# Lu-Zhan/Pano-NeRF

Hardware: AMD Instinct MI355X
Metric: rays/sec (train step) (higher is better)
Workload: dtype f32 (2xfp16 split products, fp32 accumulate; weight-gradient operands h_l / delta_l / r_l / hdot_l stored with 16 significant bits, 'Q24')

## Files before the change

### pano-nerf_amd/csrc/pn_chain.hip

```cpp
#include "pn_common.h"
#include <math.h>
#include <string.h>
#include <stdlib.h>
#include <type_traits>
#include <utility>
#include <vector>

template <typename F, int... Is>
__device__ __forceinline__ void static_for_impl(F&& f, std::integer_sequence<int, Is...>) {
    (f(std::integral_constant<int, Is>{}), ...);
}
template <int N, typename F>
__device__ __forceinline__ void static_for(F&& f) {
    static_for_impl(static_cast<F&&>(f), std::make_integer_sequence<int, N>{});
}

typedef __bf16 bf16x8 __attribute__((ext_vector_type(8)));
typedef _Float16 f16x8 __attribute__((ext_vector_type(8)));
typedef __attribute__((address_space(3))) void* lds_ptr_t;
typedef const __attribute__((address_space(1))) void* gbl_ptr_t;

#ifndef PN_CHAIN_TILE
#define PN_CHAIN_TILE 16
#endif
#ifndef PN_ABL_CHAIN
#define PN_ABL_CHAIN 0
#endif
#define HALF_PI_F 1.5707963705062866f
constexpr int TILE = PN_CHAIN_TILE;
static_assert(TILE == 16 || TILE == 32, "PN_CHAIN_TILE is 16 or 32");
constexpr int NG = 64 / TILE;
constexpr int QB = 4 * NG;
constexpr int KSTEP = 2 * QB;
constexpr int ACCQ = TILE / QB;
constexpr int ACCR = 4 * ACCQ;
#ifndef PN_CHAIN_WAVES
#define PN_CHAIN_WAVES (PN_CHAIN_TILE == 16 ? 8 : 4)
#endif
constexpr int CH_WAVES = PN_CHAIN_WAVES;
constexpr int CH_THREADS = 64 * CH_WAVES;
constexpr int CH_SAMPLES = CH_WAVES * TILE;
constexpr int CH_WG_PER_CU = (TILE == 16 && CH_WAVES == 4) ? 2 : 1;
constexpr int CH_MIN_WAVES = CH_WAVES * CH_WG_PER_CU / 4;
typedef float accv __attribute__((ext_vector_type(ACCR)));
constexpr int KS_H = 256 / KSTEP, NT_H = 256 / TILE;
constexpr int KS_ENC = 96 / KSTEP, NT_ENC = 96 / TILE;
constexpr int KS_PAD = 32 / KSTEP;
constexpr int KS_C = 128 / KSTEP, NT_C = 128 / TILE;

template <int NP>
struct Cfg {
#ifdef PN_CHAIN_CF
    static constexpr int CF = PN_CHAIN_CF;
#else
    static constexpr int CF = NP >= 2 ? 24 : (CH_WG_PER_CU == 2 ? 16 : 32);
#endif
    static constexpr int PER = CF / NP;
    static constexpr int SLOT = (CF + 1) * 1024;
#ifdef PN_CHAIN_NSLOT
    static constexpr int NSLOT = PN_CHAIN_NSLOT;
#else
    static constexpr int NSLOT = CH_WG_PER_CU == 2 ? 3 : (NP >= 2 ? 5 : 4);
#endif
    static constexpr int D = NSLOT - 1;
    static constexpr int SHARE = CF / CH_WAVES;
    static constexpr int LDS_BYTES = SLOT * NSLOT;
};

template <int NP>
struct TEl {
    typedef float type;
};
template <>
struct TEl<1> {
    typedef __bf16 type;
};
#define TP(p) reinterpret_cast<TE*>(p)
template <int NP>
struct PlaneOf {
    typedef bf16x8 type;
};
template <>
struct PlaneOf<2> {
    typedef f16x8 type;
};
template <int NP>
struct BFrag {
    typename PlaneOf<NP>::type p[NP];
};

__host__ __device__ constexpr int feat(int qb, int g, int i) { return QB * qb + 4 * g + i; }
__host__ __device__ constexpr int kmap(int ks, int g, int j) { return feat(2 * ks + (j >> 2), g, j & 3); }

enum {
    F_L0 = 0, F_L1, F_L2, F_L3, F_L4, F_L5, F_L5E, F_L6, F_L7, F_DEN, F_EXTRA, F_VIEW, F_COLOR, F_COUNT
};
enum {
    B_COLOR = 0, B_VIEW, B_EXTRA, B_L7, B_L6, B_L5, B_L4, B_L3, B_L2, B_L1, B_DENC0, B_DENC1, B_COUNT
};
__host__ __device__ constexpr int fwd_ks(int i) {
    return (i == F_L0 || i == F_L5E) ? KS_ENC : i == F_VIEW ? KS_H + KS_PAD : i == F_COLOR ? KS_C : KS_H;
}
__host__ __device__ constexpr int fwd_nt(int i) { return (i == F_DEN || i == F_COLOR) ? 1 : i == F_VIEW ? NT_C : NT_H; }
__host__ __device__ constexpr int bwd_ks(int i) {
    return i == B_COLOR ? 1 : i == B_VIEW ? KS_C : i == B_EXTRA ? KS_H + 1 : KS_H;
}
__host__ __device__ constexpr int bwd_nt(int i) { return i == B_COLOR ? NT_C : (i == B_DENC0 || i == B_DENC1) ? NT_ENC : NT_H; }
template <int NP>
__host__ __device__ constexpr int chunks_of(int KS, int NT) { return (KS * NT + Cfg<NP>::PER - 1) / Cfg<NP>::PER; }
template <int NP>
__host__ __device__ constexpr int fwd_chunk0(int i) {
    int c = 0;
    for (int k = 0; k < i; ++k) c += chunks_of<NP>(fwd_ks(k), fwd_nt(k));
    return c;
}
template <int NP>
__host__ __device__ constexpr int bwd_chunk0(int i) {
    int c = 0;
    for (int k = 0; k < i; ++k) c += chunks_of<NP>(bwd_ks(k), bwd_nt(k));
    return c;
}

struct PackSeg {
    int64_t off;
    int ld;
    int k0, kvalid;
    int transposed;
    int col0;
};
struct PackLayer {
    int chunk0, KS, NT;
    int rows_valid;
    int nseg;
    PackSeg seg[2];
    int64_t aux_off;
    int aux_n;
};
#define PACK_MAXL 32
struct PackTable {
    PackLayer L[PACK_MAXL];
    int n, nchunks;
};

constexpr int EXP_TOP = 15;
constexpr int EXP_CAP = 80;
constexpr int EXP_CAP_W = 30;
constexpr int EXP_CAP_Z = 120;
__device__ __forceinline__ int scale_exp(float amax, int cap = EXP_CAP) {
    const int e = EXP_TOP - __builtin_amdgcn_frexp_expf(amax);
    return e > cap ? cap : e;
}
constexpr int WEXP_SLICES = 16;
__global__ void k_chain_wexp(PackTable tab, const float* params, uint32_t* wmax) {
    const PackLayer& L = tab.L[blockIdx.x];
    float m = 0.f;
    for (int s = 0; s < L.nseg; ++s) {
        const PackSeg& sg = L.seg[s];
        const int n = L.rows_valid * sg.kvalid;
        for (int idx = threadIdx.x + blockDim.x * blockIdx.y; idx < n; idx += blockDim.x * WEXP_SLICES) {
            const int i = idx / sg.kvalid, kr = idx - i * sg.kvalid;
            const float x = sg.transposed ? params[sg.off + (int64_t)kr * sg.ld + sg.col0 + i]
                                          : params[sg.off + (int64_t)i * sg.ld + sg.col0 + kr];
            m = fmaxf(m, fabsf(x));
        }
    }
    __shared__ float red[256];
    red[threadIdx.x] = m;
    __syncthreads();
    for (int o = 128; o > 0; o >>= 1) {
        if ((int)threadIdx.x < o) red[threadIdx.x] = fmaxf(red[threadIdx.x], red[threadIdx.x + o]);
        __syncthreads();
    }
    if (threadIdx.x == 0) wmax[blockIdx.x * WEXP_SLICES + blockIdx.y] = __float_as_uint(red[0]);
}

template <int NP>
__global__ void k_chain_pack(PackTable tab, const float* params, unsigned char* out, int* wexp) {
    constexpr int CF = Cfg<NP>::CF, SLOT = Cfg<NP>::SLOT, PER = Cfg<NP>::PER;
    const int64_t gid = (int64_t)blockIdx.x * blockDim.x + threadIdx.x;
    const int lane = (int)(gid & 63);
    const int64_t fi = gid >> 6;
    const int chunk = (int)(fi / (CF + 1)), f = (int)(fi % (CF + 1));
    if (chunk >= tab.nchunks) return;
    int li = 0;
    for (int i = 1; i < tab.n; ++i)
        if (chunk >= tab.L[i].chunk0) li = i;
    const PackLayer& L = tab.L[li];
    unsigned char* dst = out + (int64_t)chunk * SLOT + f * 1024 + lane * 16;
    if (f == CF) {
        float v[4] = {0.f, 0.f, 0.f, 0.f};
        if (chunk == L.chunk0 + (L.KS * L.NT + PER - 1) / PER - 1 && L.aux_off >= 0)
            for (int q = 0; q < 4; ++q)
                if (lane * 4 + q < L.aux_n) v[q] = params[L.aux_off + lane * 4 + q];
        memcpy(dst, v, 16);
        return;
    }
    const int p = f % NP;
    const int step = (chunk - L.chunk0) * PER + f / NP;
    int wex = 0;
    if constexpr (NP == 2) {
        const uint32_t* wm = reinterpret_cast<const uint32_t*>(wexp) + 32 + li * WEXP_SLICES;
        uint32_t top = 0u;
#pragma unroll
        for (int sl = 0; sl < WEXP_SLICES; ++sl) top = wm[sl] > top ? wm[sl] : top;
        wex = scale_exp(__uint_as_float(top), EXP_CAP_W);
        if (chunk == L.chunk0 && f == 0 && lane == 0) wexp[li] = wex;
    }
    unsigned short o[8] = {0, 0, 0, 0, 0, 0, 0, 0};
    if (step < L.KS * L.NT) {
        const int ks = step / L.NT, tt = step % L.NT;
        const int i = TILE * tt + (lane % TILE), g = lane / TILE;
        for (int j = 0; j < 8; ++j) {
            const int k = kmap(ks, g, j);
            float x = 0.f;
            if (i < L.rows_valid)
                for (int s = 0; s < L.nseg; ++s) {
                    const PackSeg& sg = L.seg[s];
                    const int kr = k - sg.k0;
                    if (kr >= 0 && kr < sg.kvalid)
                        x = sg.transposed ? params[sg.off + (int64_t)kr * sg.ld + sg.col0 + i]
                                          : params[sg.off + (int64_t)i * sg.ld + sg.col0 + kr];
                }
            unsigned short bits;
            if constexpr (NP == 2) {
                const float t = ldexpf(x, wex);
                const _Float16 hh = (_Float16)t;
                const _Float16 r = p == 0 ? hh : (_Float16)(t - (float)hh);
                __builtin_memcpy(&bits, &r, 2);
            } else {
                const __bf16 hb = (__bf16)x;
                __bf16 r = hb;
                if (p >= 1) {
                    const float r1 = x - (float)hb;
                    const __bf16 mb = (__bf16)r1;
                    r = mb;
                    if (p == 2) r = (__bf16)(r1 - (float)mb);
                }
                __builtin_memcpy(&bits, &r, 2);
            }
            o[j] = bits;
        }
    }
    memcpy(dst, o, 16);
}

#if defined(PN_TRACE_CHAIN) || defined(PN_TRACE_WG)
__device__ unsigned long long g_chain_trace[64];
extern "C" int pn_chain_trace_read(unsigned long long* out) {
    return hipMemcpyFromSymbol(out, HIP_SYMBOL(g_chain_trace), sizeof(unsigned long long) * 64) == hipSuccess ? 0 : -4;
}
#endif
#ifdef PN_TRACE_CHAIN
#define TR(i)                                                                                          \
    do {                                                                                               \
        if (blockIdx.x == 0 && threadIdx.x == 0 && st == (int64_t)gridDim.x) g_chain_trace[i] = __builtin_amdgcn_s_memtime(); \
    } while (0)
#define TRX(i)                                                                                 \
    do {                                                                                       \
        if (blockIdx.x == 0 && threadIdx.x == 0) g_chain_trace[i] = __builtin_amdgcn_s_memtime(); \
    } while (0)
#else
#define TR(i)
#define TRX(i)
#endif

template <int NP>
struct Ring {
    static constexpr int CF = Cfg<NP>::CF, SLOT = Cfg<NP>::SLOT;
    static constexpr int PIECES = CF / CH_WAVES + 1;
    __amdgpu_buffer_rsrc_t rsrc;
    unsigned char* lds;
    uint32_t lds_addr;
    int nchunk;
    int pf, pslot, cslot;
    int wid, lane;
    int cur_soff;
    unsigned char* cur_lds;
    __device__ __forceinline__ void begin_round() {
        cur_soff = pf * SLOT;
        cur_lds = lds + pslot * SLOT;
        pf = (pf + 1 == nchunk) ? 0 : pf + 1;
        pslot = (pslot + 1 == Cfg<NP>::NSLOT) ? 0 : pslot + 1;
    }
    template <int I, bool AUX>
    __device__ __forceinline__ void piece() {
        if constexpr (I < CF / CH_WAVES) {
            const int f = wid + CH_WAVES * I;
            __builtin_amdgcn_raw_ptr_buffer_load_lds(rsrc, (lds_ptr_t)(cur_lds + f * 1024), 16, lane * 16, cur_soff + f * 1024, 0, 0);
        } else if constexpr (I == CF / CH_WAVES && AUX) {
            if (wid < 4) {
                const int o = CF * 1024 + wid * 256;
                __builtin_amdgcn_raw_ptr_buffer_load_lds(rsrc, (lds_ptr_t)(cur_lds + o), 4, lane * 4, cur_soff + o, 0, 0);
            }
        }
    }
    template <int I0, int STRIDE, bool AUX = true>
    __device__ __forceinline__ void pieces_from() {
        if constexpr (I0 < PIECES) {
            piece<I0, AUX>();
            pieces_from<I0 + STRIDE, STRIDE, AUX>();
        }
    }
    __device__ __forceinline__ void start(const unsigned char* s, unsigned char* l, int n, int w, int ln, int first) {
        rsrc = __builtin_amdgcn_make_buffer_rsrc((void*)s, 0, n * SLOT, 0x00020000);
        lds = l; nchunk = n; wid = w; lane = ln;
        lds_addr = (uint32_t)(uintptr_t)(lds_ptr_t)l;
        pf = first; pslot = 0; cslot = 0;
#pragma unroll
        for (int i = 0; i < Cfg<NP>::D; ++i) {
            begin_round();
            pieces_from<0, 1, true>();
        }
    }
#ifdef PN_TRACE_CHAIN
    unsigned long long t_lds = 0, t_dma = 0, t_bar = 0, n_acq = 0;
#endif
    __device__ __forceinline__ uint32_t acquire() {
        constexpr int N = Cfg<NP>::SHARE * (Cfg<NP>::D - 1);
#ifdef PN_TRACE_CHAIN
        const unsigned long long t0 = __builtin_amdgcn_s_memtime();
        asm volatile("s_waitcnt lgkmcnt(0)" ::: "memory");
        const unsigned long long t1 = __builtin_amdgcn_s_memtime();
        asm volatile("s_waitcnt vmcnt(%0) lgkmcnt(0)" ::"n"(N) : "memory");
        const unsigned long long t2 = __builtin_amdgcn_s_memtime();
        __builtin_amdgcn_s_barrier();
        const unsigned long long t3 = __builtin_amdgcn_s_memtime();
        asm volatile("s_waitcnt lgkmcnt(0)" ::: "memory");
        t_lds += t1 - t0; t_dma += t2 - t1; t_bar += t3 - t2; ++n_acq;
#else
        asm volatile("s_waitcnt vmcnt(%0) lgkmcnt(0)" ::"n"(N) : "memory");
        if constexpr (!(PN_ABL_CHAIN & 8)) __builtin_amdgcn_s_barrier();
#endif
        begin_round();
        const uint32_t p = lds_addr + cslot * SLOT;
        cslot = (cslot + 1 == Cfg<NP>::NSLOT) ? 0 : cslot + 1;
        return p;
    }
    __device__ __forceinline__ void drain() {
        asm volatile("s_waitcnt vmcnt(0)" ::: "memory");
        __builtin_amdgcn_s_barrier();
#ifdef PN_TRACE_CHAIN
        if (blockIdx.x == 0 && threadIdx.x == 0) {
            g_chain_trace[56] = t_lds; g_chain_trace[57] = t_dma; g_chain_trace[58] = t_bar; g_chain_trace[59] = n_acq;
        }
#endif
    }
};

__device__ __forceinline__ void chain_prio(int wid) {
#ifdef PN_CHAIN_PRIO
    if (wid >= CH_WAVES / 2) __builtin_amdgcn_s_setprio(PN_CHAIN_PRIO);
#endif
}

__device__ __forceinline__ accv mfma1(const bf16x8& a, const bf16x8& b, accv v) {
#if PN_CHAIN_TILE == 32
    return __builtin_amdgcn_mfma_f32_32x32x16_bf16(a, b, v, 0, 0, 0);
#else
    return __builtin_amdgcn_mfma_f32_16x16x32_bf16(a, b, v, 0, 0, 0);
#endif
}
__device__ __forceinline__ accv mfma1(const f16x8& a, const f16x8& b, accv v) {
#if PN_CHAIN_TILE == 32
    return __builtin_amdgcn_mfma_f32_32x32x16_f16(a, b, v, 0, 0, 0);
#else
    return __builtin_amdgcn_mfma_f32_16x16x32_f16(a, b, v, 0, 0, 0);
#endif
}
template <int NP>
__device__ __forceinline__ accv mfma_split(const BFrag<NP>& a, const BFrag<NP>& b, accv v) {
    if constexpr (NP == 3) {
        v = mfma1(a.p[2], b.p[0], v);
        v = mfma1(a.p[0], b.p[2], v);
        v = mfma1(a.p[1], b.p[1], v);
        v = mfma1(a.p[1], b.p[0], v);
        v = mfma1(a.p[0], b.p[1], v);
        v = mfma1(a.p[0], b.p[0], v);
    } else if constexpr (NP == 2) {
        v = mfma1(a.p[1], b.p[0], v);
        v = mfma1(a.p[0], b.p[1], v);
        v = mfma1(a.p[0], b.p[0], v);
    } else {
        v = mfma1(a.p[0], b.p[0], v);
    }
    return v;
}

template <int NP, int IDX>
__device__ __forceinline__ void read_a(BFrag<NP>& a, uint32_t addr) {
#pragma unroll
    for (int p = 0; p < NP; ++p)
        asm volatile("ds_read_b128 %0, %1 offset:%2" : "=v"(a.p[p]) : "v"(addr), "n"((IDX * NP + p) * 1024) : "memory");
}
template <int NP, int LEFT>
__device__ __forceinline__ void wait_a(BFrag<NP>& a) {
    if constexpr (NP == 3)
        asm volatile("s_waitcnt lgkmcnt(%3)" : "+v"(a.p[0]), "+v"(a.p[1]), "+v"(a.p[2]) : "n"(LEFT) : "memory");
    else if constexpr (NP == 2)
        asm volatile("s_waitcnt lgkmcnt(%2)" : "+v"(a.p[0]), "+v"(a.p[1]) : "n"(LEFT) : "memory");
    else
        asm volatile("s_waitcnt lgkmcnt(%1)" : "+v"(a.p[0]) : "n"(LEFT) : "memory");
}
template <int NP, int NT>
struct Unit {
    static constexpr int U = 1;
};
template <int NP>
struct Look {
    static constexpr int N = NP == 3 ? 1 : 3;
};
template <int NP>
__host__ __device__ constexpr int chunk_steps(int S, int c) {
    return (c == (S - 1) / Cfg<NP>::PER && S % Cfg<NP>::PER) ? S % Cfg<NP>::PER : Cfg<NP>::PER;
}
template <int NP, int S, int PP>
__device__ __forceinline__ void read_step(Ring<NP>& R, uint32_t& sa, int lane, BFrag<NP>& f) {
    if constexpr (PP < S) {
        if constexpr (PP % Cfg<NP>::PER == 0) sa = R.acquire() + lane * 16;
        if constexpr (PN_ABL_CHAIN & 2) f = BFrag<NP>{};
        else read_a<NP, PP % Cfg<NP>::PER>(f, sa);
    }
}
template <int NP, int S, int PP, bool BIASNEXT>
__device__ __forceinline__ void piece_step(Ring<NP>& R) {
    if constexpr (PP < S && !(PN_ABL_CHAIN & 1)) {
        constexpr int PER = Cfg<NP>::PER, c = PP / PER, n = (S + PER - 1) / PER;
        R.template pieces_from<PP % PER, chunk_steps<NP>(S, c), true>();
    }
}
template <int NP>
__device__ __forceinline__ void tie(BFrag<NP>& a) {
    if constexpr (NP == 3) asm volatile("" : "+v"(a.p[0]), "+v"(a.p[1]), "+v"(a.p[2]));
    else if constexpr (NP == 2) asm volatile("" : "+v"(a.p[0]), "+v"(a.p[1]));
    else asm volatile("" : "+v"(a.p[0]));
}
__device__ __forceinline__ void mfma_pair(const BFrag<2>& a0, const BFrag<2>& a1, const BFrag<2>& b, accv& v0, accv& v1) {
    v0 = mfma1(a0.p[1], b.p[0], v0);
    v1 = mfma1(a1.p[1], b.p[0], v1);
    v0 = mfma1(a0.p[0], b.p[1], v0);
    v1 = mfma1(a1.p[0], b.p[1], v1);
    v0 = mfma1(a0.p[0], b.p[0], v0);
    v1 = mfma1(a1.p[0], b.p[0], v1);
}
template <int NP, int KS, int NT, int S0, bool BIASNEXT, bool ZERO = false>
struct GemmStep {
    static constexpr int LA = Look<NP>::N, U = Unit<NP, NT>::U;
    static_assert(LA >= U && LA % U == 0 && (KS * NT) % U == 0, "look-ahead in whole units");
    static __device__ __forceinline__ void run(Ring<NP>& R, const BFrag<NP> (&b)[KS], accv (&acc)[NT], uint32_t& sa,
                                               BFrag<NP> (&q)[LA], int lane) {
        constexpr int S = KS * NT;
        constexpr int hi = (S0 + LA + U) < S ? (S0 + LA + U) : S;
        constexpr int young = hi > S0 + U ? hi - (S0 + U) : 0;
        BFrag<NP> nw[U];
        read_step<NP, S, S0 + LA>(R, sa, lane, nw[0]);
        if constexpr (U == 2) read_step<NP, S, S0 + LA + 1>(R, sa, lane, nw[1]);
        wait_a<NP, NP * young>(q[0]);
        constexpr int ks = S0 / NT, t = S0 % NT;
        if constexpr (U == 2) {
            tie<NP>(q[1]);
            mfma_pair(q[0], q[1], b[ks], acc[t], acc[t + 1]);
        } else if constexpr (!(PN_ABL_CHAIN & 4)) {
            if constexpr (ZERO && ks == 0) {
                accv z;
#pragma unroll
                for (int e = 0; e < ACCR; ++e) z[e] = 0.f;
                acc[t] = mfma_split<NP>(q[0], b[ks], z);
            } else {
                acc[t] = mfma_split<NP>(q[0], b[ks], acc[t]);
            }
        }
#ifdef PN_ABL_FILL
        {
            float f0 = __int_as_float(lane), f1 = f0;
#pragma unroll
            for (int k = 0; k < PN_ABL_FILL; ++k) asm volatile("v_fma_f32 %0, %1, %1, %0" : "+v"(f0) : "v"(f1));
            asm volatile("" ::"v"(f0));
        }
#endif
        __builtin_amdgcn_sched_barrier(0);
        piece_step<NP, S, S0 + LA, BIASNEXT>(R);
        if constexpr (U == 2) piece_step<NP, S, S0 + LA + 1, BIASNEXT>(R);
        __builtin_amdgcn_sched_barrier(0);
        if constexpr (S0 + U < S) {
#pragma unroll
            for (int i = 0; i + U < LA; ++i) q[i] = q[i + U];
#pragma unroll
            for (int u = 0; u < U; ++u) q[LA - U + u] = nw[u];
            GemmStep<NP, KS, NT, S0 + U, BIASNEXT, ZERO>::run(R, b, acc, sa, q, lane);
        }
    }
};
template <int NP, int S, int I, bool BIASNEXT>
__device__ __forceinline__ void gemm_prologue(Ring<NP>& R, uint32_t sa, BFrag<NP> (&q)[Look<NP>::N]) {
    if constexpr (I < Look<NP>::N && I < S) {
        read_a<NP, I>(q[I], sa);
        piece_step<NP, S, I, BIASNEXT>(R);
        gemm_prologue<NP, S, I + 1, BIASNEXT>(R, sa, q);
    }
}
template <int NP, int KS, int NT, bool BIAS, bool ZERO, bool BIASNEXT = false>
__device__ __forceinline__ void chain_gemm(Ring<NP>& R, const BFrag<NP> (&b)[KS], accv (&acc)[NT], int lane, int sc = 0) {
    constexpr int CF = Cfg<NP>::CF;
    static_assert(Look<NP>::N <= Cfg<NP>::PER, "the look-ahead stays within one chunk boundary");
    const uint32_t s0 = R.acquire();
    if constexpr (!ZERO && NP == 2) {
#pragma unroll
        for (int t = 0; t < NT; ++t)
#pragma unroll
            for (int e = 0; e < ACCR; ++e) {
                const float x = acc[t][e];
                acc[t][e] = ldexpf(x, sc);
            }
    }
    uint32_t sa = s0 + lane * 16;
    BFrag<NP> q[Look<NP>::N];
    gemm_prologue<NP, KS * NT, 0, BIASNEXT>(R, sa, q);
    GemmStep<NP, KS, NT, 0, BIASNEXT, ZERO>::run(R, b, acc, sa, q, lane);
    if constexpr (BIAS) {
        const float* aux = reinterpret_cast<const float*>(R.lds + ((sa - lane * 16) - R.lds_addr) + CF * 1024) + 4 * (lane / TILE);
        const float inv = NP == 2 ? ldexpf(1.0f, -sc) : 1.0f;
#pragma unroll
        for (int t = 0; t < NT; ++t)
#pragma unroll
            for (int qd = 0; qd < ACCQ; ++qd) {
                const f32x4 v = *reinterpret_cast<const f32x4*>(aux + QB * (ACCQ * t + qd));
#pragma unroll
                for (int i = 0; i < 4; ++i) {
                    const float x = acc[t][4 * qd + i];
                    acc[t][4 * qd + i] = NP == 2 ? __builtin_fmaf(x, inv, v[i]) : x + v[i];
                }
            }
    } else if constexpr (NP == 2) {
#pragma unroll
        for (int t = 0; t < NT; ++t)
#pragma unroll
            for (int e = 0; e < ACCR; ++e) {
                const float x = acc[t][e];
                acc[t][e] = ldexpf(x, -sc);
            }
    }
}

__device__ __forceinline__ void split2_pair(float x0, float x1, float s, uint32_t& h, uint32_t& l) {
    asm("v_fma_mixlo_f16 %0, %1, %2, 0" : "=v"(h) : "v"(x0), "v"(s));
    asm("v_fma_mixhi_f16 %0, %1, %2, 0" : "+v"(h) : "v"(x1), "v"(s));
    asm("v_fma_mixlo_f16 %0, %1, %2, -%3 op_sel_hi:[0,0,1]" : "=v"(l) : "v"(x0), "v"(s), "v"(h));
    asm("v_fma_mixhi_f16 %0, %1, %2, -%3 op_sel:[0,0,1] op_sel_hi:[0,0,1]" : "+v"(l) : "v"(x1), "v"(s), "v"(h));
}
template <int N>
__device__ __forceinline__ void split2_pairs(const float (&x)[2 * N], float s, uint32_t (&h)[N], uint32_t (&l)[N]) {
#pragma unroll
    for (int q = 0; q < N; ++q) asm("v_fma_mixlo_f16 %0, %1, %2, 0" : "=v"(h[q]) : "v"(x[2 * q]), "v"(s));
#pragma unroll
    for (int q = 0; q < N; ++q) asm("v_fma_mixhi_f16 %0, %1, %2, 0" : "+v"(h[q]) : "v"(x[2 * q + 1]), "v"(s));
#pragma unroll
    for (int q = 0; q < N; ++q)
        asm("v_fma_mixlo_f16 %0, %1, %2, -%3 op_sel_hi:[0,0,1]" : "=v"(l[q]) : "v"(x[2 * q]), "v"(s), "v"(h[q]));
#pragma unroll
    for (int q = 0; q < N; ++q)
        asm("v_fma_mixhi_f16 %0, %1, %2, -%3 op_sel:[0,0,1] op_sel_hi:[0,0,1]" : "+v"(l[q]) : "v"(x[2 * q + 1]), "v"(s), "v"(h[q]));
}
__device__ __forceinline__ float pow2f(int e) { return __int_as_float((127 + e) << 23); }
template <int NP>
__device__ __forceinline__ void split_into(const float (&x)[8], BFrag<NP>& f, int ex = 0) {
    if constexpr (NP == 2) {
        typedef uint32_t u32x4 __attribute__((ext_vector_type(4)));
        const float s = pow2f(ex);
        uint32_t hq[4], lq[4];
        split2_pairs<4>(x, s, hq, lq);
        u32x4 h, l;
#pragma unroll
        for (int q = 0; q < 4; ++q) {
            h[q] = hq[q];
            l[q] = lq[q];
        }
        f.p[0] = __builtin_bit_cast(f16x8, h);
        f.p[1] = __builtin_bit_cast(f16x8, l);
    }
    if constexpr (NP != 2) {
#pragma unroll
        for (int j = 0; j < 8; ++j) {
            const __bf16 h = (__bf16)x[j];
            f.p[0][j] = h;
            if constexpr (NP == 3) {
                const float r1 = x[j] - (float)h;
                const __bf16 m = (__bf16)r1;
                f.p[1][j] = m;
                f.p[2][j] = (__bf16)(r1 - (float)m);
            }
        }
    }
}
struct Ex {
    int ex;
    uint32_t top;
};
__device__ __forceinline__ void swap32(uint32_t x, uint32_t& a, uint32_t& b) {
    const auto r = __builtin_amdgcn_permlane32_swap(x, x, false, false);
    a = r[0];
    b = r[1];
}
__device__ __forceinline__ void swap16(uint32_t x, uint32_t& a, uint32_t& b) {
    const auto r = __builtin_amdgcn_permlane16_swap(x, x, false, false);
    a = r[0];
    b = r[1];
}
__device__ __forceinline__ float col_max(float m) {
    uint32_t a, b;
    swap32(__float_as_uint(m), a, b);
    uint32_t u = a > b ? a : b;
    if constexpr (NG == 4) {
        swap16(u, a, b);
        u = a > b ? a : b;
    }
    return __uint_as_float(u);
}
__device__ __forceinline__ float col_sum(float v) {
    uint32_t a, b;
    swap32(__float_as_uint(v), a, b);
    v = __uint_as_float(a) + __uint_as_float(b);
    if constexpr (NG == 4) {
        swap16(__float_as_uint(v), a, b);
        v = __uint_as_float(a) + __uint_as_float(b);
    }
    return v;
}
__device__ __forceinline__ uint32_t row_umax(uint32_t v) {
    uint32_t o;
    o = (uint32_t)__builtin_amdgcn_update_dpp(0, (int)v, 0xB1, 0xF, 0xF, true);
    v = v > o ? v : o;
    o = (uint32_t)__builtin_amdgcn_update_dpp(0, (int)v, 0x4E, 0xF, 0xF, true);
    v = v > o ? v : o;
    o = (uint32_t)__builtin_amdgcn_update_dpp(0, (int)v, 0x141, 0xF, 0xF, true);
    v = v > o ? v : o;
    o = (uint32_t)__builtin_amdgcn_update_dpp(0, (int)v, 0x140, 0xF, 0xF, true);
    v = v > o ? v : o;
    return v;
}
__device__ __forceinline__ Ex ex_of(float lane_max, int cap = EXP_CAP) {
    const float cm = col_max(lane_max);
    Ex e;
    e.ex = scale_exp(cm, cap);
    uint32_t v = row_umax(__float_as_uint(cm));
    if constexpr (NG == 2) {
        const uint32_t o = (uint32_t)__shfl_xor((int)v, 16, 64);
        v = v > o ? v : o;
    }
    e.top = (uint32_t)__builtin_amdgcn_readfirstlane((int)v);
    return e;
}
template <int N>
struct RunMax {
    uint32_t v[N];
    __device__ __forceinline__ void clear() {
#pragma unroll
        for (int k = 0; k < N; ++k) v[k] = 0u;
    }
    __device__ __forceinline__ void upd(int idx, uint32_t x) {
#pragma unroll
        for (int k = 0; k < N; ++k) v[k] = (idx == k && x > v[k]) ? x : v[k];
    }
    __device__ __forceinline__ void flush(uint32_t* slots, int lane, int wid, unsigned char* lds) const {
        if (!slots) return;
        uint32_t* w = reinterpret_cast<uint32_t*>(lds);
        if (lane == 0) {
#pragma unroll
            for (int k = 0; k < N; ++k) w[wid * N + k] = v[k];
        }
        __syncthreads();
        if (wid == 0 && lane < N) {
            uint32_t m = w[lane];
#pragma unroll
            for (int i = 1; i < CH_WAVES; ++i) m = m > w[i * N + lane] ? m : w[i * N + lane];
            if (m > __atomic_load_n(slots + lane, __ATOMIC_RELAXED)) atomicMax(slots + lane, m);
        }
    }
};
enum {
    AM_ENC = 0, AM_ACT0 = 1 , AM_DELTA0 = 11 ,
    AM_D8B = 19, AM_D8D = 20, AM_DHV = 21, AM_DRGB = 22, AM_RS0 = 23 , AM_TANG0 = 31 ,
    AM_EDOT = 39, AM_COEF = 40, AM_COUNT = 64
};
template <int NT>
__device__ __forceinline__ float lane_amax(const accv (&acc)[NT]) {
    float m[4] = {0.f, 0.f, 0.f, 0.f};
#pragma unroll
    for (int t = 0; t < NT; ++t)
#pragma unroll
        for (int e = 0; e < ACCR; ++e) {
            const float x = acc[t][e];
            m[e & 3] = fmaxf(m[e & 3], fabsf(x));
        }
    return fmaxf(fmaxf(m[0], m[1]), fmaxf(m[2], m[3]));
}
#define AQ(acc, qb, i) (acc)[(qb) / ACCQ][4 * ((qb) % ACCQ) + (i)]
template <int NP, int NT, int KB>
__device__ __forceinline__ void split_acc(const accv (&acc)[NT], BFrag<NP> (&b)[KB], int ex) {
#pragma unroll
    for (int s = 0; s < NT * ACCQ / 2; ++s) {
        float x[8];
#pragma unroll
        for (int j = 0; j < 8; ++j) x[j] = AQ(acc, 2 * s + (j >> 2), j & 3);
        split_into<NP>(x, b[s], ex);
    }
}
template <int NP, int NT, int KB>
__device__ __forceinline__ Ex acc_to_b(const accv (&acc)[NT], BFrag<NP> (&b)[KB], float also = 0.f, int cap = EXP_CAP) {
    constexpr int KS = NT * ACCQ / 2;
    static_assert((NT * ACCQ) % 2 == 0 && KS <= KB, "quad blocks");
    Ex e{0, 0u};
    if constexpr (NP == 2) e = ex_of(fmaxf(lane_amax<NT>(acc), also), cap);
    split_acc<NP, NT, KB>(acc, b, e.ex);
    return e;
}
#ifndef PN_T_NT
#define PN_T_NT 1
#endif
template <int NT, typename TE>
__device__ __forceinline__ void store_t(TE* base, const accv (&acc)[NT]) {
    if constexpr (PN_ABL_CHAIN & 16) return;
#pragma unroll
    for (int qb = 0; qb < NT * ACCQ; ++qb)
#pragma unroll
        for (int i = 0; i < 4; ++i) {
            const float x = AQ(acc, qb, i);
#if PN_T_NT
            __builtin_nontemporal_store((TE)x, base + (QB * qb + i) * TILE);
#else
            base[(QB * qb + i) * TILE] = (TE)x;
#endif
        }
}

#ifndef PN_NO_Q24
#define PN_NO_Q24 0
#endif
template <int NP>
constexpr bool kQ24 = (NP == 2 && TILE == 16 && !PN_NO_Q24);
__host__ __device__ constexpr bool q24_act(int slot) { return slot <= 6; }
__host__ __device__ constexpr bool q24_delta(int slot) { return slot != 0 && slot != 5; }
typedef uint32_t u32x3 __attribute__((ext_vector_type(3)));
__device__ __forceinline__ u32x3 pack_q24(float x0, float x1, float x2, float x3) {
    const uint32_t e0 = __float_as_uint(x0) + 0x80u, e1 = __float_as_uint(x1) + 0x80u;
    const uint32_t e2 = __float_as_uint(x2) + 0x80u, e3 = __float_as_uint(x3) + 0x80u;
    u32x3 v;
    v[0] = __builtin_amdgcn_perm(e1, e0, 0x05030201u);
    v[1] = __builtin_amdgcn_perm(e2, e1, 0x06050302u);
    v[2] = __builtin_amdgcn_perm(e3, e2, 0x07060503u);
    return v;
}
__device__ __forceinline__ int q24_lane(int c, int g) { return g * 192 + c * 12; }
#ifndef PN_Q24_NT
#define PN_Q24_NT 1
#endif
template <int NT>
__device__ __forceinline__ void store_q24(unsigned char* base, const accv (&acc)[NT]) {
    if constexpr (PN_ABL_CHAIN & 16) return;
#pragma unroll
    for (int qb = 0; qb < NT * ACCQ; ++qb)
#if PN_Q24_NT
        __builtin_nontemporal_store(pack_q24(AQ(acc, qb, 0), AQ(acc, qb, 1), AQ(acc, qb, 2), AQ(acc, qb, 3)), reinterpret_cast<u32x3*>(base + qb * 768));
#else
        *reinterpret_cast<u32x3*>(base + qb * 768) = pack_q24(AQ(acc, qb, 0), AQ(acc, qb, 1), AQ(acc, qb, 2), AQ(acc, qb, 3));
#endif
}

constexpr int MW = 4 / (NG / 2);
__host__ __device__ constexpr int gate_word(int ks, int j) { return (4 * ks + (j >> 1)) >> 4; }
__host__ __device__ constexpr int gate_bit(int ks, int j) { return ((4 * ks + (j >> 1)) & 15) + 16 * (j & 1); }
struct Gate {
    uint32_t w[MW];
};
template <int NT>
__device__ __forceinline__ void relu(accv (&acc)[NT]) {
#pragma unroll
    for (int t = 0; t < NT; ++t)
#pragma unroll
        for (int e = 0; e < ACCR; ++e) {
            const float x = acc[t][e];
            acc[t][e] = fmaxf(x, 0.f);
        }
}
template <int NP, int KS, int KB>
__device__ __forceinline__ void gate_words(const BFrag<NP> (&b)[KB], Gate& g) {
    typedef uint32_t u32x4 __attribute__((ext_vector_type(4)));
#pragma unroll
    for (int i = 0; i < MW; ++i) g.w[i] = 0u;
    uint32_t one = 0x00010001u;
    asm volatile("" : "+v"(one));
#pragma unroll
    for (int ks = 0; ks < KS; ++ks) {
        const u32x4 h = __builtin_bit_cast(u32x4, b[ks].p[0]);
#pragma unroll
        for (int q = 0; q < 4; ++q) {
            const uint32_t hq = h[q];
            uint32_t m;
            asm("v_pk_min_u16 %0, %1, %2" : "=v"(m) : "v"(hq), "v"(one));
            asm("v_lshl_or_b32 %0, %1, %2, %0" : "+v"(g.w[(4 * ks + q) >> 4]) : "v"(m), "n"((4 * ks + q) & 15));
        }
    }
}
template <int NT>
__device__ __forceinline__ void gate_bits(accv (&acc)[NT], const Gate& g) {
#pragma unroll
    for (int qb = 0; qb < NT * ACCQ; ++qb)
#pragma unroll
        for (int i = 0; i < 4; ++i) {
            const int ks = qb >> 1, j = 4 * (qb & 1) + i;
            const int m = __builtin_amdgcn_sbfe((int)g.w[gate_word(ks, j)], gate_bit(ks, j), 1);
            const float x = AQ(acc, qb, i);
            AQ(acc, qb, i) = __int_as_float(__float_as_int(x) & m);
        }
}
__device__ __forceinline__ Gate load_gate(const uint32_t* masks, int64_t slot, int64_t Mp, int64_t row, int g) {
    Gate r;
    const uint32_t* p = masks + ((slot * Mp + row) * 8 + MW * g);
    if constexpr (MW == 4) {
        const uint4 v = *reinterpret_cast<const uint4*>(p);
        r.w[0] = v.x; r.w[1] = v.y; r.w[2] = v.z; r.w[3] = v.w;
    } else {
        const uint2 v = *reinterpret_cast<const uint2*>(p);
        r.w[0] = v.x; r.w[1] = v.y;
    }
    return r;
}
__device__ __forceinline__ void store_gate(uint32_t* masks, int64_t slot, int64_t Mp, int64_t row, int g, const Gate& r) {
    uint32_t* p = masks + ((slot * Mp + row) * 8 + MW * g);
    if constexpr (MW == 4) *reinterpret_cast<uint4*>(p) = make_uint4(r.w[0], r.w[1], r.w[2], r.w[3]);
    else *reinterpret_cast<uint2*>(p) = make_uint2(r.w[0], r.w[1]);
}
template <int N>
__device__ __forceinline__ Gate pop_front(Gate (&q)[N]) {
    const Gate m = q[0];
#pragma unroll
    for (int i = 0; i + 1 < N; ++i) q[i] = q[i + 1];
    return m;
}


__device__ __forceinline__ float ch_sp_d1(float x) { return x > 20.f ? 1.f : 1.f / (1.f + expf(-x)); }
__device__ __forceinline__ float ch_sp_d2(float x) {
    if (x > 20.f) return 0.f;
    const float s = 1.f / (1.f + expf(-x));
    return s * (1.f - s);
}
__device__ __forceinline__ float sel3(const float (&v)[3], int ch) { return ch == 0 ? v[0] : (ch == 1 ? v[1] : v[2]); }

__device__ __forceinline__ float red_turns(float y, int& quadrant) {
    const float c_hi = 0.15915494f;
    const float c_lo = 6.4206382e-9f;
    const float p = y * c_hi;
    float e = __builtin_fmaf(y, c_hi, -p);
    e = __builtin_fmaf(y, c_lo, e);
    const float f = (p - __builtin_rintf(p)) + e;
    const float q4 = f * 4.0f;
    const float qn = __builtin_rintf(q4);
    quadrant = (int)qn;
    return (q4 - qn) * 1.5707963267948966f;
}
__device__ __forceinline__ float ksin(float x) {
    const float z = x * x;
    float p = __builtin_fmaf(z, 2.7557319e-6f, -1.9841270e-4f);
    p = __builtin_fmaf(z, p, 8.3333333e-3f);
    p = __builtin_fmaf(z, p, -1.6666667e-1f);
    return __builtin_fmaf(x * z, p, x);
}
__device__ __forceinline__ float kcos(float x) {
    const float z = x * x;
    float p = __builtin_fmaf(z, -2.7557319e-7f, 2.4801587e-5f);
    p = __builtin_fmaf(z, p, -1.3888889e-3f);
    p = __builtin_fmaf(z, p, 4.1666667e-2f);
    p = __builtin_fmaf(z, p, -0.5f);
    return __builtin_fmaf(z, p, 1.0f);
}
__device__ __forceinline__ float fast_sin(float y) {
    int q;
    const float r = red_turns(y, q);
    const float sv = ksin(r), cv = kcos(r);
    const float v = (q & 1) ? cv : sv;
    return (q & 2) ? -v : v;
}
__device__ __forceinline__ float fast_cos(float y) {
    int q;
    const float r = red_turns(y, q);
    const float sv = ksin(r), cv = kcos(r);
    const float v = (q & 1) ? sv : cv;
    return ((q + 1) & 2) ? -v : v;
}

__device__ __forceinline__ int opaque(int v) {
    asm volatile("" : "+v"(v));
    return v;
}
__device__ __forceinline__ void level_of(int f, int& l, int& ch) {
    l = (f * 43691) >> 17;
    ch = f - 3 * l;
}
__device__ __forceinline__ float pow2i(int l) { return __int_as_float((127 + l) << 23); }

struct Tile {
    int64_t blk, row, rc;
    int c, g, lo;
    bool live;
};
__device__ __forceinline__ Tile tile_of(int64_t st, int wid, int lane, int64_t M) {
    Tile t;
    t.c = lane % TILE;
    t.g = lane / TILE;
    t.blk = st * CH_WAVES + wid;
    t.row = t.blk * TILE + t.c;
    t.live = t.row < M;
    t.rc = t.live ? t.row : M - 1;
    t.lo = t.c + 4 * t.g * TILE;
    return t;
}
template <int NP, int NT>
__device__ __forceinline__ void store_vec(typename TEl<NP>::type* slot, const Tile& T, int F, bool q, const accv (&acc)[NT]) {
    if constexpr (kQ24<NP>) {
        if (q) {
            store_q24<NT>(reinterpret_cast<unsigned char*>(slot) + T.blk * (int64_t)(F * TILE * 3) + opaque(q24_lane(T.c, T.g)), acc);
            return;
        }
    }
    store_t<NT>(slot + T.blk * (int64_t)(F * TILE) + opaque(T.lo), acc);
}

template <int NP, int MODE>
__device__ __forceinline__ Ex encode(const float (&mu)[3], const float (&cv)[3], const float (&vv)[3], int g,
                                      typename TEl<NP>::type* et, BFrag<NP> (&benc)[KS_ENC]) {
    typedef typename TEl<NP>::type TE;
    constexpr int NQ = 96 / QB;
    float x[NQ][4];
    const int g4 = 4 * opaque(g);
#pragma unroll
    for (int qb = 0; qb < NQ / 2; ++qb)
#pragma unroll
        for (int i = 0; i < 4; ++i) {
            int l, ch;
            level_of(QB * qb + g4 + i, l, ch);
            const float sc = pow2i(l);
            const float y = sel3(mu, ch) * sc;
            const float e0 = __expf(-0.5f * (sel3(cv, ch) * (sc * sc)));
            if constexpr (MODE == 0) {
                x[qb][i] = e0 * fast_sin(y);
                x[qb + NQ / 2][i] = e0 * fast_sin(y + HALF_PI_F);
            } else {
                const float e = e0 * sc * sel3(vv, ch);
                x[qb][i] = e * fast_cos(y);
                x[qb + NQ / 2][i] = e * fast_cos(y + HALF_PI_F);
            }
        }
#ifdef PN_TRACE_CHAIN
#pragma unroll
    for (int qb = 0; qb < NQ; ++qb)
#pragma unroll
        for (int i = 0; i < 4; ++i) asm volatile("" ::"v"(x[qb][i]));
    if (MODE == 0) TRX(31);
#endif
#pragma unroll
    for (int qb = 0; qb < NQ; ++qb)
#pragma unroll
        for (int i = 0; i < 4; ++i) et[(QB * qb + i) * TILE] = (TE)x[qb][i];
    if (MODE == 0) TRX(32);
    Ex e{0, 0u};
    if constexpr (NP == 2) {
        if constexpr (MODE == 0) {
            e.ex = EXP_TOP - 1;
            e.top = 0x3f800000u;
        } else {
            float m = 0.f;
#pragma unroll
            for (int qb = 0; qb < NQ; ++qb)
#pragma unroll
                for (int i = 0; i < 4; ++i) m = fmaxf(m, fabsf(x[qb][i]));
            e = ex_of(m, EXP_CAP_Z);
        }
    }
#pragma unroll
    for (int s = 0; s < KS_ENC; ++s) {
        float y8[8];
#pragma unroll
        for (int j = 0; j < 8; ++j) y8[j] = x[2 * s + (j >> 2)][j & 3];
        split_into<NP>(y8, benc[s], e.ex);
    }
    return e;
}
template <int NP, int KS>
__device__ __forceinline__ int reload_b(const typename TEl<NP>::type* src, BFrag<NP> (&b)[KS], int cap = EXP_CAP) {
    if constexpr (NP == 2) {
        float x[KS][8];
        float m = 0.f;
#pragma unroll
        for (int ks = 0; ks < KS; ++ks)
#pragma unroll
            for (int j = 0; j < 8; ++j) {
                x[ks][j] = (float)src[(QB * (2 * ks + (j >> 2)) + (j & 3)) * TILE];
                m = fmaxf(m, fabsf(x[ks][j]));
            }
        const int ex = scale_exp(col_max(m), cap);
#pragma unroll
        for (int ks = 0; ks < KS; ++ks) split_into<NP>(x[ks], b[ks], ex);
        return ex;
    } else {
#pragma unroll
        for (int ks = 0; ks < KS; ++ks) {
            float x[8];
#pragma unroll
            for (int j = 0; j < 8; ++j) x[j] = (float)src[(QB * (2 * ks + (j >> 2)) + (j & 3)) * TILE];
            split_into<NP>(x, b[ks]);
        }
        return 0;
    }
}
__device__ __forceinline__ void ipe_backward_tiles(const accv (&acc)[NT_ENC], const float (&mu)[3], const float (&cv)[3], int g,
                                                   float (&dm)[3]) {
    dm[0] = dm[1] = dm[2] = 0.f;
    const int g4 = 4 * opaque(g);
#pragma unroll
    for (int qb = 0; qb < 96 / QB; ++qb)
#pragma unroll
        for (int i = 0; i < 4; ++i) {
            const bool cosine = qb >= 96 / QB / 2;
            int l, ch;
            level_of(QB * (cosine ? qb - 96 / QB / 2 : qb) + g4 + i, l, ch);
            const float sc = pow2i(l);
            const float y = sel3(mu, ch) * sc;
            const float ex = __expf(-0.5f * (sel3(cv, ch) * (sc * sc))) * sc;
            const float d = AQ(acc, qb, i) * ex * fast_cos(cosine ? y + HALF_PI_F : y);
            dm[0] += ch == 0 ? d : 0.f;
            dm[1] += ch == 1 ? d : 0.f;
            dm[2] += ch == 2 ? d : 0.f;
        }
#pragma unroll
    for (int i = 0; i < 3; ++i) {
        dm[i] = col_sum(dm[i]);
    }
}
template <int NP>
__device__ __forceinline__ Ex finish_gated(accv (&acc)[NT_H], const Gate& m, typename TEl<NP>::type* slot, const Tile& T, bool q24,
                                           BFrag<NP> (&bh)[KS_H]) {
    gate_bits<NT_H>(acc, m);
    if (slot) store_vec<NP, NT_H>(slot, T, 256, q24, acc);
    return acc_to_b<NP, NT_H, KS_H>(acc, bh, 0.f, EXP_CAP_Z);
}

__global__ void k_view_table(int64_t view_rows, const float* viewdirs, float* tab, uint32_t* amax, int amax_n) {
    if (amax && blockIdx.x == 0 && (int)threadIdx.x < amax_n) amax[threadIdx.x] = 0u;
    const int64_t idx = (int64_t)blockIdx.x * blockDim.x + threadIdx.x;
    if (idx >= view_rows * 32) return;
    const int64_t r = idx >> 5;
    const int v = (int)(idx & 31);
    const float vd0 = viewdirs[r * 3], vd1 = viewdirs[r * 3 + 1], vd2 = viewdirs[r * 3 + 2];
    auto vsel = [&](int ch) { return ch == 0 ? vd0 : (ch == 1 ? vd1 : vd2); };
    const int i = v - 3, half = i >= 12 ? 1 : 0;
    int l, ch;
    level_of(i < 0 ? 0 : i - 12 * half, l, ch);
    const float xb = vsel(ch) * pow2i(l & 3);
    const float sv = fast_sin(half ? xb + HALF_PI_F : xb);
    tab[idx] = v < 3 ? vsel(v) : (v < PN_VIEW_DIM ? sv : 0.f);
}

struct FwdArgs {
    int64_t M, nst;
    int rows_per_ray, nc;
    int64_t view_rows;
    const unsigned char* pack;
    const int* wexp;
    uint32_t* amax;
    const float* mean;
    const float* cov;
    const float* viewdirs;
    float* view_tab;
    float* enc_t;
    float* acts_t;
    uint32_t* masks;
    float* raw_rgb;
    float* raw_den;
    int q24;
};
__host__ __device__ constexpr int64_t act_off(int slot, int64_t Mp) {
    return slot <= 8 ? (int64_t)slot * Mp * 256 : 8 * Mp * 256 + Mp * 288;
}
__host__ __device__ constexpr int64_t acts_floats(int64_t Mp) { return 8 * Mp * 256 + Mp * 288 + Mp * 128; }

template <int NP>
__global__ __launch_bounds__(CH_THREADS, CH_MIN_WAVES) void k_chain_fwd(FwdArgs a) {
    extern __shared__ __attribute__((aligned(16))) unsigned char lds[];
    typedef typename TEl<NP>::type TE;
    const int tid = threadIdx.x, lane = tid & 63;
    const int wid = __builtin_amdgcn_readfirstlane(tid >> 6);
    const int64_t Mp = a.nst * CH_SAMPLES;
    chain_prio(wid);
    Ring<NP> R;
    R.start(a.pack, lds, fwd_chunk0<NP>(F_COUNT), wid, lane, 0);
    RunMax<10> RM;
    RM.clear();
#ifdef PN_TRACE_CHAIN
    if (blockIdx.x == 0 && threadIdx.x == 0) {
        g_chain_trace[60] = __builtin_amdgcn_s_memtime();
        g_chain_trace[61] = __builtin_amdgcn_s_memrealtime();
    }
#endif
    int wtab = 0;
    if constexpr (NP == 2) wtab = a.wexp[lane & 15];
    for (int64_t st = blockIdx.x; st < a.nst; st += gridDim.x) {
        const Tile T = tile_of(st, wid, lane, a.M);
        TR(0);
        TE* et = TP(a.enc_t) + T.blk * (96 * TILE) + T.lo;
        BFrag<NP> bh[KS_H];
        accv acc[NT_H];
        Gate mw;
        int bex = 0;
        auto wx = [&](int i) {
            if constexpr (NP == 2) return __builtin_amdgcn_readlane(wtab, i);
            else return 0;
        };
        {
            float mu[3], cv[3];
            const float zero3[3] = {0.f, 0.f, 0.f};
#pragma unroll
            for (int i = 0; i < 3; ++i) {
                mu[i] = a.mean[T.rc * 3 + i];
                cv[i] = a.cov[T.rc * 3 + i];
            }
            BFrag<NP> benc[KS_ENC];
#ifdef PN_TRACE_CHAIN
            asm volatile("" ::"v"(mu[0]), "v"(mu[1]), "v"(mu[2]), "v"(cv[0]), "v"(cv[1]), "v"(cv[2]));
            TRX(30);
#endif
            bex = encode<NP, 0>(mu, cv, zero3, T.g, et, benc).ex;
            TR(1);
            chain_gemm<NP, KS_ENC, NT_H, true, true, true>(R, benc, acc, lane, wx(F_L0) + bex);
            TR(2);
        }
        auto finish_hidden = [&](int slot) {
            relu<NT_H>(acc);
            if (TP(a.acts_t)) store_vec<NP, NT_H>(TP(a.acts_t) + act_off(slot, Mp), T, 256, a.q24 && q24_act(slot), acc);
            const Ex e = acc_to_b<NP, NT_H, KS_H>(acc, bh);
            gate_words<NP, KS_H, KS_H>(bh, mw);
            store_gate(a.masks, slot, Mp, T.blk * TILE + T.c, T.g, mw);
            bex = e.ex;
            RM.upd(slot, e.top);
        };
        finish_hidden(0);
        TR(3);
#pragma unroll 1
        for (int l = 1; l <= 4; ++l) {
            chain_gemm<NP, KS_H, NT_H, true, true, true>(R, bh, acc, lane, wx(F_L0 + l) + bex);
            TR(2 + 2 * l);
            finish_hidden(l);
            TR(3 + 2 * l);
        }
        {
            chain_gemm<NP, KS_H, NT_H, false, true, true>(R, bh, acc, lane, wx(F_L5) + bex);
            BFrag<NP> benc[KS_ENC];
            const int eex = reload_b<NP, KS_ENC>(et, benc);
            chain_gemm<NP, KS_ENC, NT_H, true, false, true>(R, benc, acc, lane, wx(F_L5E) + eex);
            TR(12);
            finish_hidden(5);
            TR(13);
        }
#pragma unroll 1
        for (int l = 6; l <= 7; ++l) {
            chain_gemm<NP, KS_H, NT_H, true, true, true>(R, bh, acc, lane, wx(F_L6 + l - 6) + bex);
            TR(2 + 2 * l);
            finish_hidden(l);
            TR(3 + 2 * l);
        }
        {
            accv ad[1];
            chain_gemm<NP, KS_H, 1, true, true, true>(R, bh, ad, lane, wx(F_DEN) + bex);
            if (T.live) {
#pragma unroll
                for (int i = 0; i < 4; ++i) {
                    const int ch = 4 * T.g + i;
                    if (ch < a.nc) a.raw_den[T.row * a.nc + ch] = ad[0][i];
                }
            }
        }
        TR(18);
        BFrag<NP> bv[KS_H + KS_PAD];
        int vex;
        {
            chain_gemm<NP, KS_H, NT_H, true, true, true>(R, bh, acc, lane, wx(F_EXTRA) + bex);
            TR(19);
            TE* bt = a.acts_t ? TP(a.acts_t) + act_off(8, Mp) + T.blk * (288 * TILE) + T.lo : nullptr;
            if (bt) store_t<NT_H>(bt, acc);
            const Ex e = acc_to_b<NP, NT_H, KS_H + KS_PAD>(acc, bv, 1.0f);
            vex = e.ex;
            RM.upd(8, e.top);
            const float* vt = a.view_tab + ((T.rc / a.rows_per_ray) % a.view_rows) * 32 + 4 * T.g;
#pragma unroll
            for (int q = 0; q < KS_PAD; ++q) {
                float x[8];
#pragma unroll
                for (int h = 0; h < 2; ++h) {
                    const f32x4 v = *reinterpret_cast<const f32x4*>(vt + QB * (2 * q + h));
#pragma unroll
                    for (int i = 0; i < 4; ++i) {
                        x[4 * h + i] = v[i];
                        if (bt) bt[(256 + QB * (2 * q + h) + i) * TILE] = (TE)v[i];
                    }
                }
                split_into<NP>(x, bv[KS_H + q], vex);
            }
        }
        TR(20);
        BFrag<NP> bc[KS_C];
        int cex;
        {
            accv av[NT_C];
            chain_gemm<NP, KS_H + KS_PAD, NT_C, true, true, true>(R, bv, av, lane, wx(F_VIEW) + vex);
            TR(21);
            Gate w4;
            relu<NT_C>(av);
            if (TP(a.acts_t)) store_t<NT_C>(TP(a.acts_t) + act_off(9, Mp) + T.blk * (128 * TILE) + T.lo, av);
            const Ex e = acc_to_b<NP, NT_C, KS_C>(av, bc);
            gate_words<NP, KS_C, KS_C>(bc, w4);
            store_gate(a.masks, 8, Mp, T.blk * TILE + T.c, T.g, w4);
            cex = e.ex;
            RM.upd(9, e.top);
        }
        TR(22);
        {
            accv ac[1];
            chain_gemm<NP, KS_C, 1, true, true, true>(R, bc, ac, lane, wx(F_COLOR) + cex);
            TR(23);
            if (T.live && T.g == 0) {
#pragma unroll
                for (int e = 0; e < 3; ++e) a.raw_rgb[T.row * 3 + e] = ac[0][e];
            }
        }
        TR(24);
    }
    R.drain();
#ifdef PN_TRACE_CHAIN
    if (blockIdx.x == 0 && threadIdx.x == 0) {
        g_chain_trace[62] = __builtin_amdgcn_s_memtime();
        g_chain_trace[63] = __builtin_amdgcn_s_memrealtime();
    }
#endif
    if constexpr (NP == 2) {
        RM.flush(a.amax ? a.amax + AM_ACT0 : nullptr, lane, wid, lds);
        if (a.amax && blockIdx.x == 0 && tid == 0) a.amax[AM_ENC] = 0x3f800000u;
    }
}

struct SweepArgs {
    int64_t M, nst;
    int nc;
    float density_bias;
    const unsigned char* pack;
    int nchunk;
    const int* wexp;
    uint32_t* amax;
    const uint32_t* masks;
    const float* raw_den;
    const float* mean;
    const float* cov;
    const float* wd0;
    const float* v;
    float* vec_t;
    int keep_all;
    float* edot_t;
    float* out3;
    float* sdot;
    int q24;
};

template <int NP>
__global__ __launch_bounds__(CH_THREADS, CH_MIN_WAVES) void k_chain_dgrad(SweepArgs a) {
    extern __shared__ __attribute__((aligned(16))) unsigned char lds[];
    typedef typename TEl<NP>::type TE;
    const int tid = threadIdx.x, lane = tid & 63;
    const int wid = __builtin_amdgcn_readfirstlane(tid >> 6);
    const int64_t Mp = a.nst * CH_SAMPLES;
    chain_prio(wid);
    Ring<NP> R;
    R.start(a.pack, lds, a.nchunk, wid, lane, 0);
    RunMax<8> RM;
    RM.clear();
    int wtab = 0;
    if constexpr (NP == 2) wtab = a.wexp[lane & 15];
    for (int64_t st = blockIdx.x; st < a.nst; st += gridDim.x) {
        const Tile T = tile_of(st, wid, lane, a.M);
        Gate mk[8];
#pragma unroll
        for (int l = 0; l < 8; ++l) mk[l] = load_gate(a.masks, 7 - l, Mp, T.blk * TILE + T.c, T.g);
        float mu[3], cv[3];
#pragma unroll
        for (int i = 0; i < 3; ++i) {
            mu[i] = a.mean[T.rc * 3 + i];
            cv[i] = a.cov[T.rc * 3 + i];
        }
        const float sgm = T.live ? ch_sp_d1(a.raw_den[T.rc * a.nc] + a.density_bias) : 0.f;
        BFrag<NP> bh[KS_H];
        int bex = 0;
        auto wx = [&](int i) {
            if constexpr (NP == 2) return __builtin_amdgcn_readlane(wtab, i);
            else return 0;
        };
        {
            const bool Q7 = kQ24<NP> && a.q24 && q24_delta(7);
            TE* rt = (a.keep_all && !Q7) ? TP(a.vec_t) + (int64_t)7 * Mp * 256 + T.blk * (256 * TILE) + T.lo : nullptr;
            unsigned char* rq = (a.keep_all && Q7) ? reinterpret_cast<unsigned char*>(TP(a.vec_t) + (int64_t)7 * Mp * 256) +
                                                         T.blk * (int64_t)(256 * TILE * 3) + q24_lane(T.c, T.g)
                                                   : nullptr;
            const Gate m7 = pop_front(mk);
            if constexpr (NP == 2) {
                float wm = 0.f;
#pragma unroll
                for (int qb = 0; qb < NT_H * ACCQ; ++qb) {
                    const f32x4 wv = *reinterpret_cast<const f32x4*>(a.wd0 + QB * qb + 4 * T.g);
                    wm = fmaxf(fmaxf(wm, fmaxf(fabsf(wv[0]), fabsf(wv[1]))), fmaxf(fabsf(wv[2]), fabsf(wv[3])));
                }
                const Ex e = ex_of(sgm * wm, EXP_CAP_Z);
                bex = e.ex;
                RM.upd(7, e.top);
            }
#pragma unroll
            for (int ks = 0; ks < KS_H; ++ks) {
                float x[8];
#pragma unroll
                for (int h = 0; h < 2; ++h) {
                    const f32x4 wv = *reinterpret_cast<const f32x4*>(a.wd0 + QB * (2 * ks + h) + 4 * T.g);
#pragma unroll
                    for (int i = 0; i < 4; ++i) {
                        const int j = 4 * h + i;
                        const uint32_t bit = (m7.w[gate_word(ks, j)] >> gate_bit(ks, j)) & 1u;
                        x[j] = bit ? sgm * wv[i] : 0.f;
                        if (rt) rt[(QB * (2 * ks + h) + i) * TILE] = (TE)x[j];
                    }
                    if constexpr (kQ24<NP>) {
                        if (rq) {
#if PN_Q24_NT
                            __builtin_nontemporal_store(pack_q24(x[4 * h], x[4 * h + 1], x[4 * h + 2], x[4 * h + 3]), reinterpret_cast<u32x3*>(rq + (2 * ks + h) * 768));
#else
                            *reinterpret_cast<u32x3*>(rq + (2 * ks + h) * 768) = pack_q24(x[4 * h], x[4 * h + 1], x[4 * h + 2], x[4 * h + 3]);
#endif
                        }
                    }
                }
                split_into<NP>(x, bh[ks], bex);
            }
        }
        accv acc[NT_H];
#pragma unroll 1
        for (int l = 7; l >= 1; --l) {
            chain_gemm<NP, KS_H, NT_H, false, true>(R, bh, acc, lane, wx(B_L7 + 7 - l) + bex);
            TE* dst = a.keep_all ? TP(a.vec_t) + (int64_t)(l - 1) * Mp * 256 : (l - 1 == 5 ? TP(a.vec_t) : nullptr);
            const Ex e = finish_gated<NP>(acc, pop_front(mk), dst, T, a.q24 && q24_delta(l - 1), bh);
            bex = e.ex;
            RM.upd(l - 1, e.top);
        }
        {
            accv a3[NT_ENC];
            chain_gemm<NP, KS_H, NT_ENC, false, true>(R, bh, a3, lane, wx(B_DENC0) + bex);
            bex = reload_b<NP, KS_H>(TP(a.vec_t) + (a.keep_all ? (int64_t)5 * Mp * 256 : 0) + T.blk * (256 * TILE) + T.lo, bh, EXP_CAP_Z);
            chain_gemm<NP, KS_H, NT_ENC, false, false>(R, bh, a3, lane, wx(B_DENC1) + bex);
            float dm[3];
            ipe_backward_tiles(a3, mu, cv, T.g, dm);
            if (T.live && T.g == 0) {
                a.out3[T.row * 3] = dm[0];
                a.out3[T.row * 3 + 1] = dm[1];
                a.out3[T.row * 3 + 2] = dm[2];
            }
        }
    }
    R.drain();
    if constexpr (NP == 2) RM.flush(a.amax ? a.amax + AM_RS0 : nullptr, lane, wid, lds);
}

template <int NP>
__global__ __launch_bounds__(CH_THREADS, CH_MIN_WAVES) void k_chain_tangent(SweepArgs a) {
    extern __shared__ __attribute__((aligned(16))) unsigned char lds[];
    typedef typename TEl<NP>::type TE;
    const int tid = threadIdx.x, lane = tid & 63;
    const int wid = __builtin_amdgcn_readfirstlane(tid >> 6);
    const int64_t Mp = a.nst * CH_SAMPLES;
    chain_prio(wid);
    Ring<NP> R;
    R.start(a.pack, lds, a.nchunk, wid, lane, 0);
    RunMax<9> RM;
    RM.clear();
    Ex e;
    int wtab = 0;
    if constexpr (NP == 2) wtab = a.wexp[lane & 15];
    for (int64_t st = blockIdx.x; st < a.nst; st += gridDim.x) {
        const Tile T = tile_of(st, wid, lane, a.M);
        Gate mk[8];
#pragma unroll
        for (int l = 0; l < 8; ++l) mk[l] = load_gate(a.masks, l, Mp, T.blk * TILE + T.c, T.g);
        TE* et = TP(a.edot_t) + T.blk * (96 * TILE) + T.lo;
        BFrag<NP> bh[KS_H];
        accv acc[NT_H];
        int bex = 0;
        auto wx = [&](int i) {
            if constexpr (NP == 2) return __builtin_amdgcn_readlane(wtab, i);
            else return 0;
        };
        {
            float mu[3], cv[3], vv[3];
#pragma unroll
            for (int i = 0; i < 3; ++i) {
                mu[i] = a.mean[T.rc * 3 + i];
                cv[i] = a.cov[T.rc * 3 + i];
                vv[i] = T.live ? a.v[T.rc * 3 + i] : 0.f;
            }
            BFrag<NP> benc[KS_ENC];
            e = encode<NP, 1>(mu, cv, vv, T.g, et, benc);
            bex = e.ex;
            RM.upd(8, e.top);
            chain_gemm<NP, KS_ENC, NT_H, false, true>(R, benc, acc, lane, wx(F_L0) + bex);
        }
        e = finish_gated<NP>(acc, pop_front(mk), TP(a.vec_t), T, a.q24 && q24_act(0), bh);
        bex = e.ex;
        RM.upd(0, e.top);
#pragma unroll 1
        for (int l = 1; l <= 4; ++l) {
            chain_gemm<NP, KS_H, NT_H, false, true>(R, bh, acc, lane, wx(F_L0 + l) + bex);
            e = finish_gated<NP>(acc, pop_front(mk), TP(a.vec_t) + (int64_t)l * Mp * 256, T, a.q24 && q24_act(l), bh);
            bex = e.ex;
            RM.upd(l, e.top);
        }
        {
            chain_gemm<NP, KS_H, NT_H, false, true>(R, bh, acc, lane, wx(F_L5) + bex);
            BFrag<NP> benc[KS_ENC];
            const int eex = reload_b<NP, KS_ENC>(et, benc, EXP_CAP_Z);
            chain_gemm<NP, KS_ENC, NT_H, false, false>(R, benc, acc, lane, wx(F_L5E) + eex);
            e = finish_gated<NP>(acc, pop_front(mk), TP(a.vec_t) + (int64_t)5 * Mp * 256, T, a.q24 && q24_act(5), bh);
            bex = e.ex;
            RM.upd(5, e.top);
        }
        chain_gemm<NP, KS_H, NT_H, false, true>(R, bh, acc, lane, wx(F_L6) + bex);
        e = finish_gated<NP>(acc, pop_front(mk), TP(a.vec_t) + (int64_t)6 * Mp * 256, T, a.q24 && q24_act(6), bh);
        bex = e.ex;
        RM.upd(6, e.top);
        chain_gemm<NP, KS_H, NT_H, false, true>(R, bh, acc, lane, wx(F_L7) + bex);
        {
            gate_bits<NT_H>(acc, pop_front(mk));
            store_t<NT_H>(TP(a.vec_t) + (int64_t)7 * Mp * 256 + T.blk * (256 * TILE) + T.lo, acc);
            if constexpr (NP == 2) RM.upd(7, ex_of(lane_amax<NT_H>(acc), EXP_CAP_Z).top);
            float sd = 0.f;
#pragma unroll
            for (int qb = 0; qb < NT_H * ACCQ; ++qb) {
                const f32x4 wv = *reinterpret_cast<const f32x4*>(a.wd0 + QB * qb + 4 * T.g);
#pragma unroll
                for (int i = 0; i < 4; ++i) sd += AQ(acc, qb, i) * wv[i];
            }
            sd = col_sum(sd);
            if (T.live && T.g == 0) a.sdot[T.row] = sd;
        }
    }
    R.drain();
    if constexpr (NP == 2) RM.flush(a.amax ? a.amax + AM_TANG0 : nullptr, lane, wid, lds);
}

struct BwdArgs {
    int64_t M, nst;
    int nc;
    float density_bias;
    const unsigned char* pack;
    int nchunk;
    const int* wexp;
    uint32_t* amax;
    const uint32_t* masks;
    const float* raw_den;
    const float* d_rgb;
    const float* d_den;
    const float* sdot;
    const float* mean;
    const float* cov;
    float* drgb_t;
    float* dhv_t;
    float* d8_t;
    float* delta_t;
    float* coef_t;
    float* d_mean;
    int q24;
};

template <int NP>
__global__ __launch_bounds__(CH_THREADS, CH_MIN_WAVES) void k_chain_bwd(BwdArgs a) {
    extern __shared__ __attribute__((aligned(16))) unsigned char lds[];
    typedef typename TEl<NP>::type TE;
    const int tid = threadIdx.x, lane = tid & 63;
    const int wid = __builtin_amdgcn_readfirstlane(tid >> 6);
    const int64_t Mp = a.nst * CH_SAMPLES;
    chain_prio(wid);
    Ring<NP> R;
    R.start(a.pack, lds, a.nchunk, wid, lane, 0);
    RunMax<12> RM;
    RM.clear();
    Ex e;
    int wtab = 0;
    if constexpr (NP == 2) wtab = a.wexp[lane & 15];
    for (int64_t st = blockIdx.x; st < a.nst; st += gridDim.x) {
        const Tile T = tile_of(st, wid, lane, a.M);
        Gate mk[9];
#pragma unroll
        for (int l = 0; l < 9; ++l) mk[l] = load_gate(a.masks, 8 - l, Mp, T.blk * TILE + T.c, T.g);
        BFrag<NP> b1[1];
        int bex = 0;
        auto wx = [&](int i) {
            if constexpr (NP == 2) return __builtin_amdgcn_readlane(wtab, i);
            else return 0;
        };
        {
            float x[8];
            TE* dt = TP(a.drgb_t) + T.blk * (32 * TILE) + T.lo;
            float m = 0.f;
#pragma unroll
            for (int j = 0; j < 8; ++j) {
                const int f = QB * (j >> 2) + 4 * T.g + (j & 3);
                x[j] = (T.live && f < 3) ? a.d_rgb[T.rc * 3 + (f < 3 ? f : 0)] : 0.f;
                dt[(QB * (j >> 2) + (j & 3)) * TILE] = (TE)x[j];
                m = fmaxf(m, fabsf(x[j]));
            }
            if constexpr (NP == 2) {
                e = ex_of(m, EXP_CAP_Z);
                bex = e.ex;
                RM.upd(11, e.top);
            }
            split_into<NP>(x, b1[0], bex);
        }
        BFrag<NP> bc[KS_C];
        {
            accv av[NT_C];
            chain_gemm<NP, 1, NT_C, false, true>(R, b1, av, lane, wx(B_COLOR) + bex);
            gate_bits<NT_C>(av, pop_front(mk));
            store_t<NT_C>(TP(a.dhv_t) + T.blk * (128 * TILE) + T.lo, av);
            e = acc_to_b<NP, NT_C, KS_C>(av, bc, 0.f, EXP_CAP_Z);
            bex = e.ex;
            RM.upd(10, e.top);
        }
        BFrag<NP> be[KS_H + 1];
        accv acc[NT_H];
        {
            chain_gemm<NP, KS_C, NT_H, false, true>(R, bc, acc, lane, wx(B_VIEW) + bex);
            TE* bt = TP(a.d8_t) + T.blk * (288 * TILE) + T.lo;
            store_t<NT_H>(bt, acc);
            const float z = a.raw_den[T.rc * a.nc] + a.density_bias;
            const float add0 = (a.sdot && T.live) ? ch_sp_d2(z) * a.sdot[T.rc] : 0.f;
            float x[8];
            float m = 0.f;
#pragma unroll
            for (int j = 0; j < 8; ++j) {
                const int ch = QB * (j >> 2) + 4 * T.g + (j & 3);
                float v = 0.f;
                if (T.live && ch < a.nc) v = a.d_den[T.rc * a.nc + ch] + (ch == 0 ? add0 : 0.f);
                x[j] = v;
                bt[(256 + QB * (j >> 2) + (j & 3)) * TILE] = (TE)v;
                m = fmaxf(m, fabsf(v));
            }
            if constexpr (NP == 2) {
                e = ex_of(lane_amax<NT_H>(acc), EXP_CAP_Z);
                const Ex ed = ex_of(m, EXP_CAP_Z);
                RM.upd(8, e.top);
                RM.upd(9, ed.top);
                bex = e.ex < ed.ex ? e.ex : ed.ex;
            }
            split_acc<NP, NT_H, KS_H + 1>(acc, be, bex);
            split_into<NP>(x, be[KS_H], bex);
            if (TP(a.coef_t)) {
                TE* ct = TP(a.coef_t) + T.blk * (32 * TILE) + T.lo;
                const float cf = T.live ? ch_sp_d1(z) : 0.f;
#pragma unroll
                for (int j = 0; j < 8; ++j) {
                    const int f = QB * (j >> 2) + 4 * T.g + (j & 3);
                    ct[(QB * (j >> 2) + (j & 3)) * TILE] = (TE)(f == 0 ? cf : 0.f);
                }
            }
        }
        BFrag<NP> bh[KS_H];
        chain_gemm<NP, KS_H + 1, NT_H, false, true>(R, be, acc, lane, wx(B_EXTRA) + bex);
        e = finish_gated<NP>(acc, pop_front(mk), TP(a.delta_t) + (int64_t)7 * Mp * 256, T, a.q24 && q24_delta(7), bh);
        bex = e.ex;
        RM.upd(7, e.top);
#pragma unroll 1
        for (int l = 7; l >= 1; --l) {
            chain_gemm<NP, KS_H, NT_H, false, true>(R, bh, acc, lane, wx(B_L7 + 7 - l) + bex);
            e = finish_gated<NP>(acc, pop_front(mk), TP(a.delta_t) + (int64_t)(l - 1) * Mp * 256, T, a.q24 && q24_delta(l - 1), bh);
            bex = e.ex;
            RM.upd(l - 1, e.top);
        }
        if (a.d_mean) {
            float mu[3], cv[3];
#pragma unroll
            for (int i = 0; i < 3; ++i) {
                mu[i] = a.mean[T.rc * 3 + i];
                cv[i] = a.cov[T.rc * 3 + i];
            }
            accv a3[NT_ENC];
            chain_gemm<NP, KS_H, NT_ENC, false, true>(R, bh, a3, lane, wx(B_DENC0) + bex);
            bex = reload_b<NP, KS_H>(TP(a.delta_t) + (int64_t)5 * Mp * 256 + T.blk * (256 * TILE) + T.lo, bh, EXP_CAP_Z);
            chain_gemm<NP, KS_H, NT_ENC, false, false>(R, bh, a3, lane, wx(B_DENC1) + bex);
            float dm[3];
            ipe_backward_tiles(a3, mu, cv, T.g, dm);
            if (T.live && T.g == 0) {
                a.d_mean[T.row * 3] = dm[0];
                a.d_mean[T.row * 3 + 1] = dm[1];
                a.d_mean[T.row * 3 + 2] = dm[2];
            }
        }
    }
    R.drain();
    if constexpr (NP == 2) {
        RM.flush(a.amax ? a.amax + AM_DELTA0 : nullptr, lane, wid, lds);
        if (a.amax && blockIdx.x == 0 && tid == 0) a.amax[AM_COEF] = 0x3f800000u;
    }
}

struct WSeg {
    const float* X;
    const float* Y;
    int64_t nhalf;
    int FX, FY;
    int bias;
    const uint32_t* ax;
    const uint32_t* ay;
};
struct WgArgs {
    WSeg seg[4];
    int nseg;
    int64_t half_total, per;
    float* slab;
    int64_t slab_stride;
    int bias;
};
constexpr int WG_MAXJ = 8;
struct WgMulti {
    WgArgs job[WG_MAXJ];
};

template <int NP>
__device__ __forceinline__ f32x16 mfma_split32(const BFrag<NP>& a, const BFrag<NP>& b, f32x16 v) {
    if constexpr (NP == 3) {
        v = __builtin_amdgcn_mfma_f32_32x32x16_bf16(a.p[2], b.p[0], v, 0, 0, 0);
        v = __builtin_amdgcn_mfma_f32_32x32x16_bf16(a.p[0], b.p[2], v, 0, 0, 0);
        v = __builtin_amdgcn_mfma_f32_32x32x16_bf16(a.p[1], b.p[1], v, 0, 0, 0);
        v = __builtin_amdgcn_mfma_f32_32x32x16_bf16(a.p[1], b.p[0], v, 0, 0, 0);
        v = __builtin_amdgcn_mfma_f32_32x32x16_bf16(a.p[0], b.p[1], v, 0, 0, 0);
        v = __builtin_amdgcn_mfma_f32_32x32x16_bf16(a.p[0], b.p[0], v, 0, 0, 0);
    } else if constexpr (NP == 2) {
        v = __builtin_amdgcn_mfma_f32_32x32x16_f16(a.p[1], b.p[0], v, 0, 0, 0);
        v = __builtin_amdgcn_mfma_f32_32x32x16_f16(a.p[0], b.p[1], v, 0, 0, 0);
        v = __builtin_amdgcn_mfma_f32_32x32x16_f16(a.p[0], b.p[0], v, 0, 0, 0);
    } else {
        v = __builtin_amdgcn_mfma_f32_32x32x16_bf16(a.p[0], b.p[0], v, 0, 0, 0);
    }
    return v;
}
#define WG_LD(p) __builtin_nontemporal_load(p)
#ifndef PN_WG_UNIT_NT
#define PN_WG_UNIT_NT 0
#endif
#if PN_WG_UNIT_NT
#define WG_LDU(p) __builtin_nontemporal_load(p)
#else
#define WG_LDU(p) (*(p))
#endif
template <int NP, int TM, int TN, int WM, int WN, bool X24 = false, bool Y24 = false>
__global__ __launch_bounds__(64 * WM * WN) void k_chain_wgrad(WgMulti multi) {
    const WgArgs& a = multi.job[blockIdx.y];
    static_assert(!(X24 || Y24) || (NP == 2 && TILE == 16), "Q24 tensors exist in fp16-pair builds with 16-sample tiles");
    static_assert(!X24 || Y24, "combinations in use: (0,0), (0,1), (1,1)");
    constexpr bool ROT = X24 || Y24;
    constexpr int NTH = 64 * WM * WN, TMW = 32 * TM * WM, TNW = 32 * TN * WN;
    constexpr int PX = TMW * 16, PY = TNW * 16;
    constexpr int BUF = NP * (PX + PY);
    typedef typename TEl<NP>::type TE;
    constexpr int PPR = 16 * (int)sizeof(TE) / 16;
    constexpr int SPP = 16 / PPR;
    constexpr int CX = X24 ? 0 : TMW * PPR, CY = Y24 ? 0 : TNW * PPR;
    constexpr int LX = X24 ? 1 : (CX + NTH - 1) / NTH, LY = Y24 ? 1 : (CY + NTH - 1) / NTH;
    constexpr int UX = X24 ? TMW : 0, UY = Y24 ? TNW : 0;
    constexpr int LU = (UX + UY + NTH - 1) / NTH;
    static_assert(UX % 64 == 0, "a wave's units are all X or all Y");
#ifndef PN_WG_UNIT_COAL
#define PN_WG_UNIT_COAL 0
#endif
    constexpr bool COAL = PN_WG_UNIT_COAL && (X24 || Y24);
    constexpr int SCR = COAL ? (NTH / 64) * 1536 : 0;
    __shared__ __attribute__((aligned(16))) unsigned short smem[2 * BUF + SCR];
    const int tid = threadIdx.x, lane = tid & 63;
    const int wid = __builtin_amdgcn_readfirstlane(tid >> 6);
    const int wm = wid / WN, wn = wid % WN;
    const int64_t h0 = (int64_t)blockIdx.x * a.per;
    if (h0 >= a.half_total) return;
    int64_t h1 = h0 + a.per;
    if (h1 > a.half_total) h1 = a.half_total;

    f32x16 acc[TM][TN];
#pragma unroll
    for (int i = 0; i < TM; ++i)
#pragma unroll
        for (int j = 0; j < TN; ++j)
#pragma unroll
            for (int e = 0; e < 16; ++e) acc[i][j][e] = 0.f;
    float bsum[LX];
#pragma unroll
    for (int i = 0; i < LX; ++i) bsum[i] = 0.f;
    float bsum4[LU > 0 ? LU : 1][4] = {};

#ifndef PN_WG_Q24_NSET
#define PN_WG_Q24_NSET 4
#endif
#ifndef PN_WG_Q24_ALT
#define PN_WG_Q24_ALT 1
#endif
#ifndef PN_WG_Q24_STEADY
#define PN_WG_Q24_STEADY 0
#endif
    constexpr int NSET = (X24 && LU == 1) ? PN_WG_Q24_NSET : ((NP <= 2 && (X24 ? 0 : LX) + (Y24 ? 0 : LY) + 3 * LU <= 4) ? 3 : 2);
    f32x4 xr[NSET][LX], yr[NSET][LY];
    f32x4 ur[NSET][LU > 0 ? LU : 1][3];
    constexpr bool ALT = PN_WG_Q24_ALT && (WM * WN == 8 && TM == 2 && TN == 4) && (X24 || Y24 || NP == 1);
    auto unit_of = [&](int i) { return tid + NTH * i; };
    float bw[NSET] = {};
    int sx[NSET] = {}, sy[NSET] = {}, unit = 0;
    auto seg_exps = [&](const WSeg& S, int& ex, int& ey) {
        ex = scale_exp(__uint_as_float(*S.ax), EXP_CAP_Z);
        ey = scale_exp(__uint_as_float(*S.ay), EXP_CAP_Z);
        int over = ex + ey - unit;
        const int rx = over < ex + 126 ? over : ex + 126;
        ex -= rx;
        ey -= over - rx;
        if (ey < -126) ey = -126;
    };
    if constexpr (NP == 2) {
        unit = 1 << 20;
        for (int i = 0; i < a.nseg; ++i) {
            const int e = scale_exp(__uint_as_float(*a.seg[i].ax), EXP_CAP_Z) + scale_exp(__uint_as_float(*a.seg[i].ay), EXP_CAP_Z);
            unit = e < unit ? e : unit;
        }
    }
    int csg = 0, cFX = a.seg[0].FX, cFY = a.seg[0].FY, csx = 0, csy = 0;
    int64_t cbase = 0, cend = a.seg[0].nhalf;
    const TE* cX = reinterpret_cast<const TE*>(a.seg[0].X);
    const TE* cY = reinterpret_cast<const TE*>(a.seg[0].Y);
    float cbw = a.seg[0].bias ? 1.f : 0.f;
    if constexpr (NP == 2) seg_exps(a.seg[0], csx, csy);
    auto load = [&](int64_t h, int set) __attribute__((always_inline)) {
        while (csg + 1 < a.nseg && h >= cend) {
            ++csg;
            const WSeg& S = a.seg[csg];
            cbase = cend;
            cend += S.nhalf;
            cX = reinterpret_cast<const TE*>(S.X);
            cY = reinterpret_cast<const TE*>(S.Y);
            cFX = S.FX;
            cFY = S.FY;
            cbw = S.bias ? 1.f : 0.f;
            if constexpr (NP == 2) seg_exps(S, csx, csy);
        }
        const int64_t hb = h - cbase;
        bw[set] = cbw;
        if constexpr (NP == 2) {
            sx[set] = csx;
            sy[set] = csy;
        }
        const int64_t blk = hb / (TILE / 16);
        const int half = (int)(hb % (TILE / 16));
        const TE* xb = cX + blk * ((int64_t)cFX * TILE) + half * 16;
        const TE* yb = cY + blk * ((int64_t)cFY * TILE) + half * 16;
        if constexpr (!X24) {
#pragma unroll
            for (int i = 0; i < LX; ++i) {
                const int idx = tid + NTH * i;
                if (CX % NTH == 0 || idx < CX) xr[set][i] = WG_LD(reinterpret_cast<const f32x4*>(xb + (idx / PPR) * TILE + (idx % PPR) * SPP));
            }
        }
        if constexpr (!Y24) {
#pragma unroll
            for (int i = 0; i < LY; ++i) {
                const int idx = tid + NTH * i;
                if (CY % NTH == 0 || idx < CY) yr[set][i] = WG_LD(reinterpret_cast<const f32x4*>(yb + (idx / PPR) * TILE + (idx % PPR) * SPP));
            }
        }
        if constexpr (X24 || Y24) {
            const unsigned char* xq = reinterpret_cast<const unsigned char*>(cX) + blk * ((int64_t)cFX * 48);
            const unsigned char* yq = reinterpret_cast<const unsigned char*>(cY) + blk * ((int64_t)cFY * 48);
#pragma unroll
            for (int i = 0; i < LU; ++i) {
                const int u = unit_of(i);
                if ((UX + UY) % NTH == 0 || u < UX + UY) {
                    if constexpr (COAL) {
                        const int u0 = u - lane;
                        const f32x4* p = reinterpret_cast<const f32x4*>(u0 < UX ? xq + u0 * 48 : yq + (u0 - UX) * 48) + lane;
                        ur[set][i][0] = WG_LD(p);
                        ur[set][i][1] = WG_LD(p + 64);
                        ur[set][i][2] = WG_LD(p + 128);
                    } else {
                        const f32x4* p = reinterpret_cast<const f32x4*>(u < UX ? xq + u * 48 : yq + (u - UX) * 48);
                        ur[set][i][0] = WG_LDU(p);
                        ur[set][i][1] = WG_LDU(p + 1);
                        ur[set][i][2] = WG_LDU(p + 2);
                    }
                }
            }
        }
    };
    auto put = [&](unsigned short* plane0, int pstride, int idx, const f32x4& v, int ex) {
        if constexpr (NP == 1) {
            const int f = idx >> 1, q = idx & 1;
            *reinterpret_cast<f32x4*>(plane0 + f * 16 + ((q ^ ((f >> 3) & 1)) << 3)) = v;
            return;
        }
        const int f0 = idx >> 2, q = idx & 3;
        const int f = ROT ? ((f0 & ~3) | ((f0 + (f0 >> 2)) & 3)) : f0;
        const int o = f * 16 + (((q >> 1) ^ ((f >> 3) & 1)) << 3) + (q & 1) * 4;
        if constexpr (NP == 2) {
            const float s = pow2f(ex);
            const float x4[4] = {v[0], v[1], v[2], v[3]};
            uint32_t h2[2], l2[2];
            split2_pairs<2>(x4, s, h2, l2);
            *reinterpret_cast<uint2*>(plane0 + o) = make_uint2(h2[0], h2[1]);
            *reinterpret_cast<uint2*>(plane0 + pstride + o) = make_uint2(l2[0], l2[1]);
        } else {
            typedef __bf16 bf16x4 __attribute__((ext_vector_type(4)));
            bf16x4 hv, mv, lv;
#pragma unroll
            for (int c = 0; c < 4; ++c) {
                const __bf16 hb = (__bf16)v[c];
                hv[c] = hb;
                if constexpr (NP == 3) {
                    const float r1 = v[c] - (float)hb;
                    const __bf16 mb = (__bf16)r1;
                    mv[c] = mb;
                    lv[c] = (__bf16)(r1 - (float)mb);
                }
            }
            *reinterpret_cast<bf16x4*>(plane0 + o) = hv;
            if constexpr (NP == 3) {
                *reinterpret_cast<bf16x4*>(plane0 + pstride + o) = mv;
                *reinterpret_cast<bf16x4*>(plane0 + 2 * pstride + o) = lv;
            }
        }
    };
    auto put_unit = [&](unsigned short* plane0, int pstride, int u, const f32x4 (&r)[3], int ex, float* bs, float w) {
        typedef uint32_t u32x4 __attribute__((ext_vector_type(4)));
        uint32_t d[12];
#pragma unroll
        for (int k = 0; k < 3; ++k) {
            const u32x4 t = __builtin_bit_cast(u32x4, r[k]);
#pragma unroll
            for (int c = 0; c < 4; ++c) d[4 * k + c] = t[c];
        }
        float e[4][4];
#pragma unroll
        for (int sm = 0; sm < 4; ++sm) {
            e[sm][0] = __uint_as_float(d[3 * sm] << 8);
            e[sm][1] = __uint_as_float(__builtin_amdgcn_perm(d[3 * sm + 1], d[3 * sm], 0x0504030cu));
            e[sm][2] = __uint_as_float(__builtin_amdgcn_perm(d[3 * sm + 2], d[3 * sm + 1], 0x0403020cu));
            e[sm][3] = __uint_as_float(d[3 * sm + 2] & 0xffffff00u);
        }
        const int qb = u >> 2, sg = u & 3;
#pragma unroll
        for (int f = 0; f < 4; ++f) {
            const f32x4 v{e[0][f], e[1][f], e[2][f], e[3][f]};
            put(plane0, pstride, (4 * qb + f) * 4 + sg, v, ex);
            if (bs) bs[f] += w * ((v[0] + v[1]) + (v[2] + v[3]));
        }
    };
#ifndef PN_ABL_WG
#define PN_ABL_WG 0
#endif
    auto stage = [&](int buf, int set) __attribute__((always_inline)) {
        unsigned short* xs = smem + buf * BUF;
        unsigned short* ys = xs + NP * PX;
        if constexpr (PN_ABL_WG & 2) {
            if constexpr (X24 || Y24) {
#pragma unroll
                for (int i = 0; i < LU; ++i) asm volatile("" ::"v"(ur[set][i][0]), "v"(ur[set][i][1]), "v"(ur[set][i][2]));
            }
            if constexpr (!X24) {
#pragma unroll
                for (int i = 0; i < LX; ++i) asm volatile("" ::"v"(xr[set][i]));
            }
            if constexpr (!Y24) {
#pragma unroll
                for (int i = 0; i < LY; ++i) asm volatile("" ::"v"(yr[set][i]));
            }
            return;
        }
        if constexpr (X24 || Y24) {
#pragma unroll
            for (int i = 0; i < LU; ++i) {
                const int u = unit_of(i);
                if ((UX + UY) % NTH == 0 || u < UX + UY) {
                    if constexpr (COAL) {
                        f32x4* scr = reinterpret_cast<f32x4*>(smem + 2 * BUF) + wid * 192;
                        scr[lane] = ur[set][i][0];
                        scr[lane + 64] = ur[set][i][1];
                        scr[lane + 128] = ur[set][i][2];
                        __builtin_amdgcn_fence(__ATOMIC_RELEASE, "wavefront");
                        __builtin_amdgcn_wave_barrier();
                        __builtin_amdgcn_fence(__ATOMIC_ACQUIRE, "wavefront");
                        f32x4 un[3];
                        un[0] = scr[3 * lane];
                        un[1] = scr[3 * lane + 1];
                        un[2] = scr[3 * lane + 2];
                        __builtin_amdgcn_wave_barrier();
                        if (u < UX) put_unit(xs, PX, u, un, sx[set], bsum4[i], bw[set]);
                        else put_unit(ys, PY, u - UX, un, sy[set], nullptr, 0.f);
                    } else {
                        if (u < UX) put_unit(xs, PX, u, ur[set][i], sx[set], bsum4[i], bw[set]);
                        else put_unit(ys, PY, u - UX, ur[set][i], sy[set], nullptr, 0.f);
                    }
                }
            }
        }
        if constexpr (!X24)
#pragma unroll
        for (int i = 0; i < LX; ++i) {
            const int idx = tid + NTH * i;
            if (CX % NTH == 0 || idx < CX) {
                put(xs, PX, idx, xr[set][i], sx[set]);
                if constexpr (NP == 1) {
                    const bf16x8 hv = __builtin_bit_cast(bf16x8, xr[set][i]);
                    float t = 0.f;
#pragma unroll
                    for (int c = 0; c < 8; ++c) t += (float)hv[c];
                    bsum[i] += bw[set] * t;
                } else {
                    bsum[i] += bw[set] * ((xr[set][i][0] + xr[set][i][1]) + (xr[set][i][2] + xr[set][i][3]));
                }
            }
        }
        if constexpr (!Y24)
#pragma unroll
        for (int i = 0; i < LY; ++i) {
            const int idx = tid + NTH * i;
            if (CY % NTH == 0 || idx < CY) put(ys, PY, idx, yr[set][i], sy[set]);
        }
    };
    const int fr = lane & 31, fh = lane >> 5;
    auto frag = [&](const unsigned short* plane, int feature) {
        if constexpr (ROT) feature = (feature & ~3) | ((feature + (feature >> 2)) & 3);
        return *reinterpret_cast<const typename PlaneOf<NP>::type*>(plane + feature * 16 + ((fh ^ ((feature >> 3) & 1)) << 3));
    };
    auto compute = [&](int buf) __attribute__((always_inline)) {
        if constexpr (PN_ABL_WG & 1) return;
        const unsigned short* xs = smem + buf * BUF;
        const unsigned short* ys = xs + NP * PX;
#ifndef PN_WG_X24_PREFETCH
#define PN_WG_X24_PREFETCH 0
#endif
        if constexpr (X24 && !PN_WG_X24_PREFETCH) {
            BFrag<NP> af[TM];
#pragma unroll
            for (int i = 0; i < TM; ++i)
#pragma unroll
                for (int p = 0; p < NP; ++p) af[i].p[p] = frag(xs + p * PX, 32 * (wm * TM + i) + fr);
#pragma unroll
            for (int j = 0; j < TN; ++j) {
                BFrag<NP> bf;
#pragma unroll
                for (int p = 0; p < NP; ++p) bf.p[p] = frag(ys + p * PY, 32 * (wn * TN + j) + fr);
#pragma unroll
                for (int i = 0; i < TM; ++i) acc[i][j] = mfma_split32<NP>(af[i], bf, acc[i][j]);
            }
            return;
        }
        typedef typename PlaneOf<NP>::type Frag;
        auto lds_of = [](const unsigned short* q) { return (uint32_t)(uintptr_t)(lds_ptr_t)q; };
        auto fidx = [&](int feature) {
            if constexpr (ROT) feature = (feature & ~3) | ((feature + (feature >> 2)) & 3);
            return feature * 16 + ((fh ^ ((feature >> 3) & 1)) << 3);
        };
        const uint32_t xa = lds_of(xs) + 2 * fidx(32 * (wm * TM) + fr), ya = lds_of(ys) + 2 * fidx(32 * (wn * TN) + fr);
        auto rd = [](Frag& dst, uint32_t addr, auto off) {
            asm volatile("ds_read_b128 %0, %1 offset:%2" : "=v"(dst) : "v"(addr), "n"(decltype(off)::value) : "memory");
        };
        static_assert(2 * NP * PX + 1024 * TM < 65536 && 2 * NP * PY + 1024 * TN < 65536, "16-bit offset field of ds_read_b128");
        BFrag<NP> af[TM];
        BFrag<NP> bf[2];
        auto read_b = [&](auto jc, BFrag<NP>& f) {
            constexpr int J = decltype(jc)::value;
            static_for<NP>([&](auto pc) {
                constexpr int P = decltype(pc)::value;
                rd(f.p[P], ya, std::integral_constant<int, 1024 * J + 2 * P * PY>{});
            });
        };
        auto settle = [&](auto left, BFrag<NP>& f) {
            constexpr int L = decltype(left)::value;
#pragma unroll
            for (int p = 0; p < NP; ++p) {
                if (p == 0) asm volatile("s_waitcnt lgkmcnt(%1)" : "+v"(f.p[p]) : "n"(L) : "memory");
                else asm volatile("" : "+v"(f.p[p]));
            }
        };
        read_b(std::integral_constant<int, 0>{}, bf[0]);
        static_for<TM>([&](auto ic) {
            constexpr int I = decltype(ic)::value;
            static_for<NP>([&](auto pc) {
                constexpr int P = decltype(pc)::value;
                rd(af[I].p[P], xa, std::integral_constant<int, 1024 * I + 2 * P * PX>{});
            });
        });
        if constexpr (TN > 1) {
            read_b(std::integral_constant<int, 1>{}, bf[1]);
            settle(std::integral_constant<int, NP>{}, bf[0]);
        } else {
            settle(std::integral_constant<int, 0>{}, bf[0]);
        }
#pragma unroll
        for (int i = 0; i < TM; ++i)
#pragma unroll
            for (int p = 0; p < NP; ++p) asm volatile("" : "+v"(af[i].p[p]));
        static_for<TN>([&](auto jc) {
            constexpr int J = decltype(jc)::value;
#pragma unroll
            for (int i = 0; i < TM; ++i) acc[i][J] = mfma_split32<NP>(af[i], bf[J & 1], acc[i][J]);
            if constexpr (J + 2 < TN) {
                __builtin_amdgcn_sched_barrier(0);
                read_b(std::integral_constant<int, J + 2>{}, bf[J & 1]);
            }
            if constexpr (J + 1 < TN) {
                if constexpr (J + 2 < TN) settle(std::integral_constant<int, NP>{}, bf[(J + 1) & 1]);
                else settle(std::integral_constant<int, 0>{}, bf[(J + 1) & 1]);
            }
        });
    };
#ifdef PN_TRACE_WG
    unsigned long long tw[4] = {0, 0, 0, 0};
#define WGT(i, expr)                                                   \
    do {                                                               \
        const unsigned long long t0_ = __builtin_amdgcn_s_memtime();   \
        expr;                                                          \
        asm volatile("s_waitcnt lgkmcnt(0)" ::: "memory");             \
        tw[i] += __builtin_amdgcn_s_memtime() - t0_;                   \
    } while (0)
#else
#define WGT(i, expr) expr
#endif
    auto one = [&](auto kc, int64_t h) __attribute__((always_inline)) {
        constexpr int K = decltype(kc)::value;
        if (h + K < h1) {
            WGT(0, stage(K % 2, K % NSET));
            WGT(1, __syncthreads());
            WGT(2, if (h + K + NSET < h1) load(h + K + NSET, K % NSET));
            WGT(3, compute(K % 2));
        }
    };
    if constexpr (ALT) {
        const int t = wid >= (WM * WN) / 2 ? 1 : 0;
        const int64_t n = h1 - h0;
        auto clampd = [&](int64_t hb) { return h0 + (hb < n ? hb : n - 1); };
        if (n > 0) {
            load(h0, 0);
            stage(0, 0);
            load(clampd(1), 0);
            if (t && 1 < n) stage(1, 0);
#pragma unroll
            for (int sidx = 1; sidx < NSET; ++sidx) load(clampd(sidx + t), sidx);
            load(clampd(NSET + t), 0);
            __syncthreads();
            constexpr int TRIPA = NSET == 3 ? 6 : (NSET == 4 ? 4 : 2);
            auto alt = [&](auto kc, auto guard, int64_t k0) __attribute__((always_inline)) {
                constexpr int K = decltype(kc)::value;
                if (!decltype(guard)::value || k0 + K < n) {
                    WGT(3, compute(K % 2));
                    if (t && !(PN_ABL_WG & 4)) WGT(1, __syncthreads());
                    const int64_t hb = k0 + K + 1 + t;
                    if (hb < n) WGT(0, stage((K + 1 + t) & 1, (K + 1) % NSET));
                    WGT(2, load(clampd(hb + NSET), (K + 1) % NSET));
                    if (!t && !(PN_ABL_WG & 4)) WGT(1, __syncthreads());
                }
            };
            int64_t k0 = 0;
            for (; k0 + TRIPA <= n; k0 += TRIPA) {
                alt(std::integral_constant<int, 0>{}, std::false_type{}, k0);
                alt(std::integral_constant<int, 1>{}, std::false_type{}, k0);
                if constexpr (TRIPA >= 4) {
                    alt(std::integral_constant<int, 2>{}, std::false_type{}, k0);
                    alt(std::integral_constant<int, 3>{}, std::false_type{}, k0);
                }
                if constexpr (TRIPA == 6) {
                    alt(std::integral_constant<int, 4>{}, std::false_type{}, k0);
                    alt(std::integral_constant<int, 5>{}, std::false_type{}, k0);
                }
            }
            if (k0 < n) {
                alt(std::integral_constant<int, 0>{}, std::true_type{}, k0);
                alt(std::integral_constant<int, 1>{}, std::true_type{}, k0);
                if constexpr (TRIPA >= 4) {
                    alt(std::integral_constant<int, 2>{}, std::true_type{}, k0);
                    alt(std::integral_constant<int, 3>{}, std::true_type{}, k0);
                }
                if constexpr (TRIPA == 6) {
                    alt(std::integral_constant<int, 4>{}, std::true_type{}, k0);
                    alt(std::integral_constant<int, 5>{}, std::true_type{}, k0);
                }
            }
        }
    } else
    if (h0 < h1) {
#pragma unroll
        for (int k = 0; k < NSET; ++k) {
            if constexpr (X24 && PN_WG_Q24_STEADY) load(h0 + k < h1 ? h0 + k : h1 - 1, k);
            else if (h0 + k < h1) load(h0 + k, k);
        }
        constexpr int TRIP = NSET == 3 ? 6 : (NSET == 4 ? 4 : 2);
        int64_t hs = h0;
        if constexpr (X24 && PN_WG_Q24_STEADY) {
            auto steady = [&](auto kc, int64_t h) __attribute__((always_inline)) {
                constexpr int K = decltype(kc)::value;
                stage(K % 2, K % NSET);
                __syncthreads();
                const int64_t hn = h + K + NSET;
                load(hn < h1 ? hn : h1 - 1, K % NSET);
                compute(K % 2);
            };
            for (; hs + TRIP <= h1; hs += TRIP) {
                steady(std::integral_constant<int, 0>{}, hs);
                steady(std::integral_constant<int, 1>{}, hs);
                if constexpr (TRIP >= 4) {
                    steady(std::integral_constant<int, 2>{}, hs);
                    steady(std::integral_constant<int, 3>{}, hs);
                }
                if constexpr (TRIP == 6) {
                    steady(std::integral_constant<int, 4>{}, hs);
                    steady(std::integral_constant<int, 5>{}, hs);
                }
            }
        }
        for (int64_t h = hs; h < h1; h += TRIP) {
            one(std::integral_constant<int, 0>{}, h);
            one(std::integral_constant<int, 1>{}, h);
            if constexpr (TRIP == 4) {
                one(std::integral_constant<int, 2>{}, h);
                one(std::integral_constant<int, 3>{}, h);
            }
            if constexpr (TRIP == 6) {
                one(std::integral_constant<int, 2>{}, h);
                one(std::integral_constant<int, 3>{}, h);
                one(std::integral_constant<int, 4>{}, h);
                one(std::integral_constant<int, 5>{}, h);
            }
        }
    }
#ifdef PN_TRACE_WG
    if (blockIdx.x == 0 && lane == 0 && (X24 && Y24)) {
#pragma unroll
        for (int i = 0; i < 4; ++i) g_chain_trace[8 * i + wid] = tw[i];
        if (wid == 0) g_chain_trace[32] = (unsigned long long)(h1 - h0);
    }
#endif
    float* out = a.slab + (int64_t)blockIdx.x * a.slab_stride;
#pragma unroll
    for (int i = 0; i < TM; ++i)
#pragma unroll
        for (int j = 0; j < TN; ++j)
#pragma unroll
            for (int e = 0; e < 16; ++e) {
                const int row = 32 * (wm * TM + i) + (e & 3) + 8 * (e >> 2) + 4 * fh;
                const float x = acc[i][j][e];
                out[(int64_t)row * TNW + 32 * (wn * TN + j) + fr] = NP == 2 ? ldexpf(x, -unit) : x;
            }
    if constexpr (X24) {
        if (a.bias) {
#pragma unroll
            for (int i = 0; i < LU; ++i) {
                const int u = tid + NTH * i;
#pragma unroll
                for (int f = 0; f < 4; ++f) {
                    float v = bsum4[i][f];
                    v += __shfl_xor(v, 1, 64);
                    v += __shfl_xor(v, 2, 64);
                    if ((u & 3) == 0 && u < UX) out[(int64_t)TMW * TNW + 4 * (u >> 2) + f] = v;
                }
            }
        }
    } else if (a.bias) {
#pragma unroll
        for (int i = 0; i < LX; ++i) {
            float v = bsum[i];
            v += __shfl_xor(v, 1, 64);
            if constexpr (PPR == 4) v += __shfl_xor(v, 2, 64);
            const int idx = tid + NTH * i;
            if (idx % PPR == 0 && (CX % NTH == 0 || idx < CX)) out[(int64_t)TMW * TNW + idx / PPR] = v;
        }
    }
}

static void fill_layer(PackLayer& L, int chunk0, int KS, int NT, int rows_valid) {
    L.chunk0 = chunk0; L.KS = KS; L.NT = NT; L.rows_valid = rows_valid;
    L.nseg = 0; L.aux_off = -1; L.aux_n = 0;
}
static void add_seg(PackLayer& L, int64_t off, int ld, int k0, int kvalid, int transposed, int col0) {
    L.seg[L.nseg++] = PackSeg{off, ld, k0, kvalid, transposed, col0};
}

template <int NP>
static PackTable fwd_table(int nc) {
    const PnLayout P = pn_layout(nc);
    PackTable T;
    T.n = F_COUNT;
    const int ld5 = PN_WIDTH + PN_ENC_DIM;
    for (int i = 0; i < F_COUNT; ++i) {
        PackLayer& L = T.L[i];
        const int KS = fwd_ks(i), NT = fwd_nt(i);
        fill_layer(L, fwd_chunk0<NP>(i), KS, NT, TILE * NT);
        if (i == F_L5) {
            add_seg(L, P.w[5], ld5, 0, PN_WIDTH, 0, 0);
        } else if (i == F_L5E) {
            add_seg(L, P.w[5], ld5, 0, PN_ENC_DIM, 0, PN_WIDTH);
            L.aux_off = P.b[5]; L.aux_n = PN_WIDTH;
        } else if (i <= F_L7) {
            const int l = i < F_L5E ? i : i - 1;
            const int k = (l == 0) ? PN_ENC_DIM : PN_WIDTH;
            add_seg(L, P.w[l], k, 0, k, 0, 0);
            L.aux_off = P.b[l]; L.aux_n = PN_WIDTH;
        } else if (i == F_DEN) {
            L.rows_valid = nc;
            add_seg(L, P.wd, PN_WIDTH, 0, PN_WIDTH, 0, 0);
            L.aux_off = P.bd; L.aux_n = nc;
        } else if (i == F_EXTRA) {
            add_seg(L, P.we, PN_WIDTH, 0, PN_WIDTH, 0, 0);
            L.aux_off = P.be; L.aux_n = PN_WIDTH;
        } else if (i == F_VIEW) {
            L.rows_valid = PN_WIDTH_COND;
            add_seg(L, P.wv, PN_WIDTH + PN_VIEW_DIM, 0, PN_WIDTH + PN_VIEW_DIM, 0, 0);
            L.aux_off = P.bv; L.aux_n = PN_WIDTH_COND;
        } else {
            L.rows_valid = 3;
            add_seg(L, P.wc, PN_WIDTH_COND, 0, PN_WIDTH_COND, 0, 0);
            L.aux_off = P.bc; L.aux_n = 3;
        }
    }
    T.nchunks = fwd_chunk0<NP>(F_COUNT);
    return T;
}

template <int NP>
static PackTable bwd_table(int nc) {
    const PnLayout P = pn_layout(nc);
    PackTable T;
    T.n = B_COUNT;
    const int ldv = PN_WIDTH + PN_VIEW_DIM, ld5 = PN_WIDTH + PN_ENC_DIM;
    for (int i = 0; i < B_COUNT; ++i) {
        PackLayer& L = T.L[i];
        const int KS = bwd_ks(i), NT = bwd_nt(i);
        fill_layer(L, bwd_chunk0<NP>(i), KS, NT, TILE * NT);
        if (i == B_COLOR) {
            L.rows_valid = PN_WIDTH_COND;
            add_seg(L, P.wc, PN_WIDTH_COND, 0, 3, 1, 0);
        } else if (i == B_VIEW) {
            add_seg(L, P.wv, ldv, 0, PN_WIDTH_COND, 1, 0);
        } else if (i == B_EXTRA) {
            add_seg(L, P.we, PN_WIDTH, 0, PN_WIDTH, 1, 0);
            add_seg(L, P.wd, PN_WIDTH, PN_WIDTH, nc, 1, 0);
        } else if (i >= B_L7 && i <= B_L1) {
            const int l = 7 - (i - B_L7);
            add_seg(L, P.w[l], l == 5 ? ld5 : PN_WIDTH, 0, PN_WIDTH, 1, 0);
        } else if (i == B_DENC0) {
            L.rows_valid = PN_ENC_DIM;
            add_seg(L, P.w[0], PN_ENC_DIM, 0, PN_WIDTH, 1, 0);
        } else {
            L.rows_valid = PN_ENC_DIM;
            add_seg(L, P.w[5], ld5, 0, PN_WIDTH, 1, PN_WIDTH);
        }
    }
    T.nchunks = bwd_chunk0<NP>(B_COUNT);
    return T;
}

template <int NP>
static constexpr int64_t chain_bytes() { return (int64_t)(fwd_chunk0<NP>(F_COUNT) + bwd_chunk0<NP>(B_COUNT)) * Cfg<NP>::SLOT; }
constexpr int64_t WEXP_BYTES = 4 * (32 + 32 * WEXP_SLICES);
static_assert(F_COUNT + B_COUNT <= 32, "wexp table: 32 exponents + 32 x WEXP_SLICES maxima");
static_assert(F_COUNT <= 16 && B_COUNT <= 16, "the chain kernels keep a direction's exponents in lanes 0..15");
template <int NP>
static int pack_both(int nc, const float* params, unsigned char* out, hipStream_t s) {
    int* wexp = reinterpret_cast<int*>(out + chain_bytes<NP>());
    PackTable T = fwd_table<NP>(nc);
    const PackTable B = bwd_table<NP>(nc);
    static_assert(F_COUNT + B_COUNT <= PACK_MAXL, "one table for both directions");
    for (int i = 0; i < B.n; ++i) {
        T.L[T.n + i] = B.L[i];
        T.L[T.n + i].chunk0 += T.nchunks;
    }
    T.n += B.n;
    T.nchunks += B.nchunks;
    if (NP == 2) {
        hipLaunchKernelGGL(k_chain_wexp, dim3(T.n, WEXP_SLICES), dim3(256), 0, s, T, params, reinterpret_cast<uint32_t*>(wexp) + 32);
        PN_CHECK_LAUNCH();
    }
    const int64_t threads = (int64_t)T.nchunks * (Cfg<NP>::CF + 1) * 64;
    hipLaunchKernelGGL(k_chain_pack<NP>, dim3((unsigned)((threads + 255) / 256)), dim3(256), 0, s, T, params, out, wexp);
    PN_CHECK_LAUNCH();
    return PN_OK;
}

static_assert(Cfg<1>::LDS_BYTES <= 160 * 1024 && Cfg<2>::LDS_BYTES <= 160 * 1024 && Cfg<3>::LDS_BYTES <= 160 * 1024,
              "the weight ring must fit a CU's 160 KB of LDS");
static_assert(PN_ROW_PAD % CH_SAMPLES == 0, "sample buffers are padded to whole workgroup tiles");
constexpr int PN_MAX_DEVICES = 64;
static int current_device() {
    int dev = 0;
    if (hipGetDevice(&dev) != hipSuccess || dev < 0 || dev >= PN_MAX_DEVICES) dev = 0;
    return dev;
}
struct AttrDone {
    bool done[PN_MAX_DEVICES];
};
template <typename K, typename A>
static int launch_chain(K kernel, int lds_bytes, AttrDone& attr, int64_t nst, int max_wgs, const A& a, hipStream_t s, int cls, double flops);

static int g_chain_cus[PN_MAX_DEVICES] = {};
static int chain_cus() {
    const int dev = current_device();
    if (!g_chain_cus[dev]) {
        hipDeviceProp_t pr;
        g_chain_cus[dev] = hipGetDeviceProperties(&pr, dev) == hipSuccess ? pr.multiProcessorCount : 256;
    }
    return g_chain_cus[dev];
}
static int chain_grid(int64_t nst, int max_wgs) {
    int64_t wgs = (int64_t)chain_cus() * CH_WG_PER_CU;
    if (max_wgs > 0 && max_wgs < wgs) wgs = max_wgs;
#ifdef PN_TRACE_CHAIN
    if (getenv("PN_TRACE_ONE_WG")) wgs = chain_cus();
#endif
    return (int)(nst < wgs ? nst : wgs);
}

template <typename K, typename A>
static int launch_chain(K kernel, int lds_bytes, AttrDone& attr, int64_t nst, int max_wgs, const A& a, hipStream_t s, int cls, double flops) {
    PnProfScope prof(cls, flops, s);
    const int dev = current_device();
    if (!attr.done[dev]) {
        if (hipFuncSetAttribute((const void*)kernel, hipFuncAttributeMaxDynamicSharedMemorySize, lds_bytes) != hipSuccess)
            return PN_ERR_HIP;
        attr.done[dev] = true;
    }
    hipLaunchKernelGGL(kernel, dim3(chain_grid(nst, max_wgs)), dim3(CH_THREADS), lds_bytes, s, a);
    PN_CHECK_LAUNCH();
    return PN_OK;
}
#define LAUNCH_CHAIN(KERNEL, planes, nst, wgs, args, s, cls, flops)                                                   \
    do {                                                                                                             \
        static AttrDone done3 = {}, done2 = {}, done1 = {};                                                          \
        if ((planes) == 3) return launch_chain(KERNEL<3>, Cfg<3>::LDS_BYTES, done3, nst, wgs, args, s, cls, flops);  \
        if ((planes) == 2) return launch_chain(KERNEL<2>, Cfg<2>::LDS_BYTES, done2, nst, wgs, args, s, cls, flops);  \
        if ((planes) == 1) return launch_chain(KERNEL<1>, Cfg<1>::LDS_BYTES, done1, nst, wgs, args, s, cls, flops);  \
        return PN_ERR_UNSUPPORTED;                                                                                   \
    } while (0)
struct ChainGeom {
    int64_t slot, bytes;
    int f_all, f_den, b_all, b_l7, b_denc0;
};
template <int NP>
static ChainGeom geom_of() {
    return ChainGeom{Cfg<NP>::SLOT, chain_bytes<NP>(), fwd_chunk0<NP>(F_COUNT), fwd_chunk0<NP>(F_DEN),
                     bwd_chunk0<NP>(B_COUNT), bwd_chunk0<NP>(B_L7), bwd_chunk0<NP>(B_DENC0)};
}
static bool chain_geom(int planes, ChainGeom& g) {
    if (planes == 3) g = geom_of<3>();
    else if (planes == 2) g = geom_of<2>();
    else if (planes == 1) g = geom_of<1>();
    else return false;
    return true;
}
static double flops_mlp(int nc) { return 2.0 * ((nc == 5 ? 611328.0 : 610304.0)); }
static const double kFlopsSweep = 1016320.0;


struct WgJob {
    WSeg seg[4];
    int nseg;
    int cfg;
    int rows, cols;
    float* dst; int ldd;
    float* dbias;
    int fmt;
};
static const int kCfgM[5] = {256, 256, 128, 32, 32};
static const int kCfgN[5] = {256, 96, 288, 256, 128};

struct RedJob {
    const float* slabs;
    int64_t nb, stride, bias_off;
    int rows, cols, src_ld, ldd;
    float* dst;
    float* dbias;
};
constexpr int RED_MAXJ = WG_MAXJ;
struct RedMulti {
    RedJob job[RED_MAXJ];
};
__global__ __launch_bounds__(256) void k_reduce_job(RedMulti multi) {
    const RedJob& J = multi.job[blockIdx.y];
    const float* slabs = J.slabs;
    const int64_t nb = J.nb, stride = J.stride;
    const int rows = J.rows, cols = J.cols;
    float* dbias = J.dbias;
    __shared__ float red[4][64];
    const int tx = threadIdx.x & 63, ty = threadIdx.x >> 6;
    const int e = blockIdx.x * 64 + tx, nw = rows * cols, n = nw + (dbias ? rows : 0);
    if (blockIdx.x * 64 >= n) return;
    float acc = 0.f;
    float* d = nullptr;
    if (e < n) {
        const float* p;
        if (e < nw) {
            const int r = e / cols, c = e - r * cols;
            p = slabs + (int64_t)r * J.src_ld + c;
            d = J.dst + (int64_t)r * J.ldd + c;
        } else {
            p = slabs + J.bias_off + (e - nw);
            d = dbias + (e - nw);
        }
        int64_t b = ty;
        float a0 = 0.f, a1 = 0.f, a2 = 0.f, a3 = 0.f, a4 = 0.f, a5 = 0.f, a6 = 0.f, a7 = 0.f;
        for (; b + 28 < nb; b += 32) {
            a0 += p[b * stride];
            a1 += p[(b + 4) * stride];
            a2 += p[(b + 8) * stride];
            a3 += p[(b + 12) * stride];
            a4 += p[(b + 16) * stride];
            a5 += p[(b + 20) * stride];
            a6 += p[(b + 24) * stride];
            a7 += p[(b + 28) * stride];
        }
        for (; b < nb; b += 4) a0 += p[b * stride];
        acc = ((a0 + a1) + (a2 + a3)) + ((a4 + a5) + (a6 + a7));
    }
    red[ty][tx] = acc;
    __syncthreads();
    if (ty == 0 && e < n) *d += (red[0][tx] + red[1][tx]) + (red[2][tx] + red[3][tx]);
}

static int run_reduce(const std::vector<RedJob>& red, size_t i0, size_t i1, hipStream_t s);
template <int NP>
static int run_wgrad_group(const WgJob* jobs, int nj, float* work, int64_t work_floats, int max_wgs, hipStream_t s) {
    int64_t used = 0;
    std::vector<RedJob> red;
    if (nj < 1 || nj > WG_MAXJ) return PN_ERR_BAD_SHAPE;
    const WgJob& j0 = jobs[0];
    const int TMW = kCfgM[j0.cfg], TNW = kCfgN[j0.cfg];
    const int64_t stride = (int64_t)TMW * TNW + TMW;
    static const int kPerCu[5] = {1, 1, 1, 3, 4};
    int cus = chain_cus();
    if (max_wgs > 0 && max_wgs < cus) cus = max_wgs;
    const int64_t slots = (int64_t)cus * kPerCu[j0.cfg] / nj;
    WgMulti m{};
    int64_t nsplit_max = 0, slab0 = 0;
    float* const base = work + used;
    double flops = 0;
    for (int q = 0; q < nj; ++q) {
        const WgJob& j = jobs[q];
        if (j.cfg != j0.cfg || j.fmt != j0.fmt) return PN_ERR_BAD_SHAPE;
        WgArgs& a = m.job[q];
        int64_t total = 0;
        for (int i = 0; i < j.nseg; ++i) {
            a.seg[i] = j.seg[i];
            total += j.seg[i].nhalf;
        }
        a.nseg = j.nseg;
        a.half_total = total;
        int64_t nsplit = slots < 1 ? 1 : slots;
        if (nsplit > (total + 3) / 4) nsplit = (total + 3) / 4;
        if (nsplit < 1) nsplit = 1;
        a.per = (total + nsplit - 1) / nsplit;
        nsplit = (total + a.per - 1) / a.per;
        a.slab = base + slab0 * stride;
        a.slab_stride = stride;
        a.bias = j.dbias != nullptr;
        red.push_back(RedJob{a.slab, nsplit, stride, (int64_t)TMW * TNW, j.rows, j.cols, TNW, j.ldd, j.dst, j.dbias});
        slab0 += nsplit;
        nsplit_max = nsplit > nsplit_max ? nsplit : nsplit_max;
        double rows = 0;
        for (int i = 0; i < j.nseg; ++i) rows += 16.0 * (double)j.seg[i].nhalf;
        flops += 2.0 * rows * j.rows * j.cols;
    }
    if (used + slab0 * stride > work_floats) return PN_ERR_BAD_SHAPE;
    used += slab0 * stride;
    const dim3 grid((unsigned)nsplit_max, (unsigned)nj);
    const WgJob& j = j0;
    const WgMulti& a = m;
    {
    PnProfScope prof((j.cfg == 0 && j.fmt) ? (j.fmt == 3 ? 12 : 11) : 6 + j.cfg, flops, s);
    switch (j.cfg) {
        case 0:
            if constexpr (kQ24<NP>) {
                if (j.fmt == 3) { hipLaunchKernelGGL((k_chain_wgrad<NP, 2, 4, 4, 2, true, true>), grid, dim3(512), 0, s, a); break; }
                if (j.fmt == 1) { hipLaunchKernelGGL((k_chain_wgrad<NP, 2, 4, 4, 2, false, true>), grid, dim3(512), 0, s, a); break; }
            }
            if (j.fmt != 0) return PN_ERR_UNSUPPORTED;
            hipLaunchKernelGGL((k_chain_wgrad<NP, 2, 4, 4, 2>), grid, dim3(512), 0, s, a);
            break;
        case 1: hipLaunchKernelGGL((k_chain_wgrad<NP, 1, 3, 8, 1>), grid, dim3(512), 0, s, a); break;
        case 2: hipLaunchKernelGGL((k_chain_wgrad<NP, 1, 3, 4, 3>), grid, dim3(768), 0, s, a); break;
        case 3: hipLaunchKernelGGL((k_chain_wgrad<NP, 1, 2, 1, 4>), grid, dim3(256), 0, s, a); break;
        default: hipLaunchKernelGGL((k_chain_wgrad<NP, 1, 1, 1, 4>), grid, dim3(256), 0, s, a); break;
    }
    }
    PN_CHECK_LAUNCH();
    return run_reduce(red, 0, red.size(), s);
}
static int run_reduce(const std::vector<RedJob>& red, size_t i0, size_t i1, hipStream_t s) {
    while (i0 < i1) {
        const size_t n = i1 - i0 < (size_t)RED_MAXJ ? i1 - i0 : (size_t)RED_MAXJ;
        RedMulti r{};
        int nmax = 0;
        for (size_t q = 0; q < n; ++q) {
            r.job[q] = red[i0 + q];
            const int e = r.job[q].rows * r.job[q].cols + (r.job[q].dbias ? r.job[q].rows : 0);
            nmax = e > nmax ? e : nmax;
        }
        hipLaunchKernelGGL(k_reduce_job, dim3((unsigned)((nmax + 63) / 64), (unsigned)n), dim3(256), 0, s, r);
        PN_CHECK_LAUNCH();
        i0 += n;
    }
    return PN_OK;
}

static bool tfmt_ok(int planes, int t_format) { return t_format == 0 || (t_format == 1 && planes == 2 && kQ24<2>); }

extern "C" {

int pn_chain_tile(void) { return TILE; }

int pn_chain_q24_slots(int planes, int t_format, int tensor) {
    if (planes != 2 || t_format != 1 || !kQ24<2> || tensor < 0 || tensor > 3) return 0;
    int m = 0;
    for (int sl = 0; sl < 8; ++sl)
        if (tensor < 2 ? q24_act(sl) : q24_delta(sl)) m |= 1 << sl;
    return m;
}

int64_t pn_chain_pack_bytes(int planes) {
    ChainGeom g;
    if (!chain_geom(planes, g)) return PN_ERR_UNSUPPORTED;
    return g.bytes + WEXP_BYTES;
}

int pn_chain_pack(const float* params, int nc, int planes, void* pack, void* stream) {
    if (nc != 1 && nc != 5) return PN_ERR_UNSUPPORTED;
    if (!params || !pack) return PN_ERR_NULL;
    hipStream_t s = (hipStream_t)stream;
    unsigned char* out = (unsigned char*)pack;
    if (planes == 3) return pack_both<3>(nc, params, out, s);
    if (planes == 2) return pack_both<2>(nc, params, out, s);
    if (planes == 1) return pack_both<1>(nc, params, out, s);
    return PN_ERR_UNSUPPORTED;
}

int64_t pn_chain_acts_floats(int64_t M) { return acts_floats(pn_pad(M)); }

int pn_chain_amax_slots(void) { return AM_COUNT; }

int pn_chain_forward(int64_t M, int rows_per_ray, int64_t view_rows, int nc, int planes, const void* pack,
                     const float* mean, const float* cov, const float* viewdirs, float* view_tab, float* enc_t, float* acts_t,
                     uint32_t* masks, float* raw_rgb, float* raw_den, uint32_t* amax, int t_format, int max_wgs, void* stream) {
    if (M <= 0 || rows_per_ray <= 0 || view_rows <= 0 || max_wgs < 0) return PN_ERR_BAD_SHAPE;
    if (!tfmt_ok(planes, t_format)) return PN_ERR_UNSUPPORTED;
    if (nc != 1 && nc != 5) return PN_ERR_UNSUPPORTED;
    if (!pack || !mean || !cov || !viewdirs || !view_tab || !enc_t || !masks || !raw_rgb || !raw_den) return PN_ERR_NULL;
    FwdArgs a{};
    a.M = M;
    a.nst = pn_pad(M) / CH_SAMPLES;
    a.rows_per_ray = rows_per_ray;
    a.nc = nc;
    a.view_rows = view_rows;
    ChainGeom g;
    if (!chain_geom(planes, g)) return PN_ERR_UNSUPPORTED;
    a.pack = (const unsigned char*)pack;
    a.wexp = reinterpret_cast<const int*>(a.pack + g.bytes);
    a.mean = mean; a.cov = cov; a.viewdirs = viewdirs; a.view_tab = view_tab;
    a.enc_t = enc_t; a.acts_t = acts_t; a.masks = masks; a.raw_rgb = raw_rgb; a.raw_den = raw_den;
    a.amax = planes == 2 ? amax : nullptr;
    a.q24 = t_format;
    static_assert(AM_COUNT <= 256, "k_view_table's first workgroup clears the table of maxima");
    hipLaunchKernelGGL(k_view_table, dim3((unsigned)((view_rows * 32 + 255) / 256)), dim3(256), 0, (hipStream_t)stream, view_rows,
                       viewdirs, view_tab, a.amax, AM_COUNT);
    PN_CHECK_LAUNCH();
    LAUNCH_CHAIN(k_chain_fwd, planes, a.nst, max_wgs, a, (hipStream_t)stream, 2, (double)M * flops_mlp(nc));
}

int pn_chain_density_grad(int64_t M, int nc, int planes, float density_bias, const float* params, const void* pack,
                          const float* mean, const float* cov, const uint32_t* masks, const float* raw_den, float* rs_t,
                          int keep_all, float* grad_mean, uint32_t* amax, int t_format, int max_wgs, void* stream) {
    if (M <= 0 || max_wgs < 0) return PN_ERR_BAD_SHAPE;
    if (!tfmt_ok(planes, t_format)) return PN_ERR_UNSUPPORTED;
    if (nc != 1 && nc != 5) return PN_ERR_UNSUPPORTED;
    ChainGeom g;
    if (!chain_geom(planes, g)) return PN_ERR_UNSUPPORTED;
    if (!params || !pack || !mean || !cov || !masks || !raw_den || !rs_t || !grad_mean) return PN_ERR_NULL;
    SweepArgs a{};
    a.M = M;
    a.nst = pn_pad(M) / CH_SAMPLES;
    a.nc = nc;
    a.density_bias = density_bias;
    a.pack = (const unsigned char*)pack + (int64_t)(g.f_all + g.b_l7) * g.slot;
    a.nchunk = g.b_all - g.b_l7;
    a.wexp = reinterpret_cast<const int*>((const unsigned char*)pack + g.bytes) + F_COUNT;
    a.masks = masks; a.raw_den = raw_den; a.mean = mean; a.cov = cov;
    a.wd0 = params + pn_layout(nc).wd;
    a.vec_t = rs_t; a.out3 = grad_mean; a.keep_all = keep_all != 0;
    a.amax = planes == 2 ? amax : nullptr;
    a.q24 = t_format;
    LAUNCH_CHAIN(k_chain_dgrad, planes, a.nst, max_wgs, a, (hipStream_t)stream, 3, (double)M * kFlopsSweep);
}

int pn_chain_tangent(int64_t M, int nc, int planes, const float* params, const void* pack, const float* mean,
                     const float* cov, const uint32_t* masks, const float* v, float* edot_t, float* tang_t, float* sdot,
                     uint32_t* amax, int t_format, int max_wgs, void* stream) {
    if (M <= 0 || max_wgs < 0) return PN_ERR_BAD_SHAPE;
    if (!tfmt_ok(planes, t_format)) return PN_ERR_UNSUPPORTED;
    if (nc != 1 && nc != 5) return PN_ERR_UNSUPPORTED;
    ChainGeom g;
    if (!chain_geom(planes, g)) return PN_ERR_UNSUPPORTED;
    if (!params || !pack || !mean || !cov || !masks || !v || !edot_t || !tang_t || !sdot) return PN_ERR_NULL;
    SweepArgs a{};
    a.M = M;
    a.nst = pn_pad(M) / CH_SAMPLES;
    a.nc = nc;
    a.pack = (const unsigned char*)pack;
    a.nchunk = g.f_den;
    a.wexp = reinterpret_cast<const int*>((const unsigned char*)pack + g.bytes);
    a.masks = masks; a.mean = mean; a.cov = cov; a.v = v;
    a.wd0 = params + pn_layout(nc).wd;
    a.vec_t = tang_t; a.edot_t = edot_t; a.sdot = sdot;
    a.amax = planes == 2 ? amax : nullptr;
    a.q24 = t_format;
    LAUNCH_CHAIN(k_chain_tangent, planes, a.nst, max_wgs, a, (hipStream_t)stream, 4, (double)M * kFlopsSweep);
}

int pn_chain_backward(int64_t M, int nc, int planes, float density_bias, const void* pack, const uint32_t* masks,
                      const float* raw_den, const float* d_raw_rgb, const float* d_raw_den, const float* sdot,
                      const float* mean, const float* cov, float* drgb_t, float* dhv_t, float* d8_t, float* delta_t,
                      float* coef_t, float* d_mean, uint32_t* amax, int t_format, int max_wgs, void* stream) {
    if (M <= 0 || max_wgs < 0) return PN_ERR_BAD_SHAPE;
    if (!tfmt_ok(planes, t_format)) return PN_ERR_UNSUPPORTED;
    if (nc != 1 && nc != 5) return PN_ERR_UNSUPPORTED;
    ChainGeom g;
    if (!chain_geom(planes, g)) return PN_ERR_UNSUPPORTED;
    if (!pack || !masks || !raw_den || !d_raw_rgb || !d_raw_den || !drgb_t || !dhv_t || !d8_t || !delta_t) return PN_ERR_NULL;
    if (d_mean && (!mean || !cov)) return PN_ERR_NULL;
    if ((sdot == nullptr) != (coef_t == nullptr)) return PN_ERR_NULL;
    BwdArgs a{};
    a.M = M;
    a.nst = pn_pad(M) / CH_SAMPLES;
    a.nc = nc;
    a.density_bias = density_bias;
    a.pack = (const unsigned char*)pack + (int64_t)g.f_all * g.slot;
    a.nchunk = d_mean ? g.b_all : g.b_denc0;
    a.wexp = reinterpret_cast<const int*>((const unsigned char*)pack + g.bytes) + F_COUNT;
    a.masks = masks; a.raw_den = raw_den; a.d_rgb = d_raw_rgb; a.d_den = d_raw_den; a.sdot = sdot;
    a.mean = mean; a.cov = cov;
    a.drgb_t = drgb_t; a.dhv_t = dhv_t; a.d8_t = d8_t; a.delta_t = delta_t; a.coef_t = coef_t; a.d_mean = d_mean;
    a.amax = planes == 2 ? amax : nullptr;
    a.q24 = t_format;
    LAUNCH_CHAIN(k_chain_bwd, planes, a.nst, max_wgs, a, (hipStream_t)stream, 5, (double)M * (flops_mlp(nc) - (d_mean ? 0.0 : 2.0 * 2 * 96 * 256)));
}


int64_t pn_chain_wgrad_work_floats(void) {
    const int64_t stride = 256 * 288 + 256;
    return (256 + 64) * stride + 1024;
}

int pn_chain_wgrad(int n, const PnChainEval* ev, int nc, int planes, float* grads, float* work, int64_t work_floats,
                   int which, int t_format, int max_wgs, void* stream) {
    if (n < 1 || n > 3 || which < 1 || which > 3 || max_wgs < 0) return PN_ERR_BAD_SHAPE;
    if (!tfmt_ok(planes, t_format)) return PN_ERR_UNSUPPORTED;
    const bool first = which & 1, second = which & 2;
    if (nc != 1 && nc != 5) return PN_ERR_UNSUPPORTED;
    if (planes != 1 && planes != 2 && planes != 3) return PN_ERR_UNSUPPORTED;
    if (!ev || !grads || !work) return PN_ERR_NULL;
    hipStream_t s = (hipStream_t)stream;
    const PnLayout L = pn_layout(nc);
    int n2 = 0;
    for (int e = 0; e < n; ++e) {
        if (ev[e].M <= 0 || !ev[e].enc_t || !ev[e].acts_t) return PN_ERR_NULL;
        if (first && (!ev[e].drgb_t || !ev[e].dhv_t || !ev[e].d8_t || !ev[e].delta_t)) return PN_ERR_NULL;
        if (ev[e].rs_t) {
            if (!ev[e].edot_t || !ev[e].tang_t || (first && !ev[e].coef_t)) return PN_ERR_NULL;
            if (second) ++n2;
        }
        if (planes == 2 && !ev[e].amax) return PN_ERR_NULL;
    }
    if ((first ? n : 0) + n2 > 4) return PN_ERR_UNSUPPORTED;
    if (!first && !n2) return PN_OK;
    std::vector<WgJob> jobs;
    std::vector<int> after;
    auto run = [&](const WgJob& j, int later = 0) {
        if (j.nseg) {
            jobs.push_back(j);
            after.push_back(later);
        }
        return (int)PN_OK;
    };
    auto am = [&](int e, int slot) -> const uint32_t* { return ev[e].amax ? ev[e].amax + slot : nullptr; };
    auto mp = [&](int e) { return pn_pad(ev[e].M); };
    const int64_t esz = planes == 1 ? 2 : 4;
    auto at = [&](const float* p, int64_t elems) { return reinterpret_cast<const float*>(reinterpret_cast<const char*>(p) + elems * esz); };
    auto act = [&](int e, int slot) { return at(ev[e].acts_t, act_off(slot, mp(e))); };
    int rc;
    for (int l = 0; l < 8; ++l) {
        WgJob j{};
        for (int e = 0; e < n; ++e) {
            const int64_t Mp = mp(e);
            if (first)
                j.seg[j.nseg++] = WSeg{at(ev[e].delta_t, (int64_t)l * Mp * 256), l == 0 ? ev[e].enc_t : act(e, l - 1), Mp / 16, 256,
                                       l == 0 ? 96 : 256, 1, am(e, AM_DELTA0 + l), am(e, l == 0 ? AM_ENC : AM_ACT0 + l - 1)};
            if (second && ev[e].rs_t)
                j.seg[j.nseg++] = WSeg{at(ev[e].rs_t, (int64_t)l * Mp * 256),
                                       l == 0 ? ev[e].edot_t : at(ev[e].tang_t, (int64_t)(l - 1) * Mp * 256), Mp / 16, 256,
                                       l == 0 ? 96 : 256, 0, am(e, AM_RS0 + l), am(e, l == 0 ? AM_EDOT : AM_TANG0 + l - 1)};
        }
        j.cfg = l == 0 ? 1 : 0;
        j.fmt = (t_format == 1 && l >= 1) ? (q24_delta(l) ? 3 : 1) : 0;
        j.rows = 256;
        j.cols = l == 0 ? 96 : 256;
        j.dst = grads + L.w[l];
        j.ldd = l == 0 ? 96 : (l == 5 ? 352 : 256);
        j.dbias = first ? grads + L.b[l] : nullptr;
        if ((rc = run(j)) != PN_OK) return rc;
        if (l == 5) {
            WgJob k{};
            for (int e = 0; e < n; ++e) {
                const int64_t Mp = mp(e);
                if (first)
                    k.seg[k.nseg++] = WSeg{at(ev[e].delta_t, (int64_t)5 * Mp * 256), ev[e].enc_t, Mp / 16, 256, 96, 0,
                                           am(e, AM_DELTA0 + 5), am(e, AM_ENC)};
                if (second && ev[e].rs_t)
                    k.seg[k.nseg++] = WSeg{at(ev[e].rs_t, (int64_t)5 * Mp * 256), ev[e].edot_t, Mp / 16, 256, 96, 0,
                                           am(e, AM_RS0 + 5), am(e, AM_EDOT)};
            }
            k.cfg = 1; k.rows = 256; k.cols = 96;
            k.dst = grads + L.w[5] + 256; k.ldd = 352; k.dbias = nullptr;
            if ((rc = run(k)) != PN_OK) return rc;
        }
    }
    if (first) {
        WgJob j{};
        for (int e = 0; e < n; ++e) j.seg[j.nseg++] = WSeg{ev[e].d8_t, act(e, 7), mp(e) / 16, 288, 256, 1, am(e, AM_D8B), am(e, AM_ACT0 + 7)};
        j.cfg = 0; j.rows = 256; j.cols = 256; j.dst = grads + L.we; j.ldd = 256; j.dbias = grads + L.be;
        if ((rc = run(j)) != PN_OK) return rc;
    }
    {
        WgJob j{};
        if (first)
            for (int e = 0; e < n; ++e) j.seg[j.nseg++] = WSeg{at(ev[e].d8_t, 256 * TILE), act(e, 7), mp(e) / 16, 288, 256, 1, am(e, AM_D8D), am(e, AM_ACT0 + 7)};
        j.cfg = 3; j.rows = nc; j.cols = 256; j.dst = grads + L.wd; j.ldd = 256; j.dbias = grads + L.bd;
        if ((rc = run(j)) != PN_OK) return rc;
        WgJob k{};
        for (int e = 0; e < n; ++e)
            if (first && ev[e].rs_t)
                k.seg[k.nseg++] = WSeg{ev[e].coef_t, at(ev[e].tang_t, (int64_t)7 * mp(e) * 256), mp(e) / 16, 32, 256, 0,
                                       am(e, AM_COEF), am(e, AM_TANG0 + 7)};
        if (k.nseg) {
            k.cfg = 3; k.rows = 1; k.cols = 256; k.dst = grads + L.wd; k.ldd = 256; k.dbias = nullptr;
            if ((rc = run(k, 1)) != PN_OK) return rc;
        }
    }
    if (first) {
        WgJob j{};
        for (int e = 0; e < n; ++e) j.seg[j.nseg++] = WSeg{ev[e].dhv_t, act(e, 8), mp(e) / 16, 128, 288, 1, am(e, AM_DHV), am(e, AM_ACT0 + 8)};
        j.cfg = 2; j.rows = 128; j.cols = PN_WIDTH + PN_VIEW_DIM; j.dst = grads + L.wv; j.ldd = PN_WIDTH + PN_VIEW_DIM;
        j.dbias = grads + L.bv;
        if ((rc = run(j)) != PN_OK) return rc;
    }
    if (first) {
        WgJob j{};
        for (int e = 0; e < n; ++e) j.seg[j.nseg++] = WSeg{ev[e].drgb_t, act(e, 9), mp(e) / 16, 32, 128, 1, am(e, AM_DRGB), am(e, AM_ACT0 + 9)};
        j.cfg = 4; j.rows = 3; j.cols = 128; j.dst = grads + L.wc; j.ldd = 128; j.dbias = grads + L.bc;
        if ((rc = run(j)) != PN_OK) return rc;
    }
    constexpr int64_t WG_RANGE = 512;
    std::vector<char> done(jobs.size(), 0);
    for (int pass = 0; pass < 2; ++pass)
    for (size_t i = 0; i < jobs.size(); ++i) {
        if (done[i] || after[i] != pass) continue;
        WgJob grp[WG_MAXJ];
        int ng = 0;
        int64_t total_i = 0;
        for (int q = 0; q < jobs[i].nseg; ++q) total_i += jobs[i].seg[q].nhalf;
        int cus_i = chain_cus();
        if (max_wgs > 0 && max_wgs < cus_i) cus_i = max_wgs;
        int64_t gmax = WG_RANGE * cus_i / (total_i > 0 ? total_i : 1);
        gmax = gmax < 1 ? 1 : (gmax > WG_MAXJ ? WG_MAXJ : gmax);
        for (size_t k = i; k < jobs.size() && ng < gmax; ++k)
            if (!done[k] && jobs[k].cfg == jobs[i].cfg && jobs[k].fmt == jobs[i].fmt && after[k] == after[i]) {
                grp[ng++] = jobs[k];
                done[k] = 1;
            }
        rc = planes == 3 ? run_wgrad_group<3>(grp, ng, work, work_floats, max_wgs, s)
                         : (planes == 2 ? run_wgrad_group<2>(grp, ng, work, work_floats, max_wgs, s)
                                        : run_wgrad_group<1>(grp, ng, work, work_floats, max_wgs, s));
        if (rc != PN_OK) return rc;
    }
    return PN_OK;
}

}
```

Baseline: 186,100.

## Let ring acquire leave pending activation stores outstanding via compile-time vmcnt slack

Chain kernels now get a store-mode template parameter (none, full-precision, Q24) chosen at launch, so whether activation and gradient stores happen is known at compile time. Each chain GEMM is told how many global stores the previous layer left in flight. The ring buffer's acquire then waits on a vmcnt that includes those stores, so it no longer drains them before the next weight chunk. This is meant to overlap tensor stores with the weight DMA and MFMA work instead of stalling at every layer boundary, at the cost of more kernel variants and exact store-count bookkeeping that silently breaks correctness or speed if a count is wrong.

```diff
diff --git a/pano-nerf_amd/csrc/pn_chain.hip b/pano-nerf_amd/csrc/pn_chain.hip
--- a/pano-nerf_amd/csrc/pn_chain.hip
+++ b/pano-nerf_amd/csrc/pn_chain.hip
@@ -25,6 +25,9 @@
 #endif
 #ifndef PN_ABL_CHAIN
 #define PN_ABL_CHAIN 0
+#endif
+#ifndef PN_RING_STORES
+#define PN_RING_STORES 1
 #endif
 #define HALF_PI_F 1.5707963705062866f
 constexpr int TILE = PN_CHAIN_TILE;
@@ -315,8 +318,10 @@
 #ifdef PN_TRACE_CHAIN
     unsigned long long t_lds = 0, t_dma = 0, t_bar = 0, n_acq = 0;
 #endif
+    template <int EXTRA = 0>
     __device__ __forceinline__ uint32_t acquire() {
-        constexpr int N = Cfg<NP>::SHARE * (Cfg<NP>::D - 1);
+        constexpr int N0 = Cfg<NP>::SHARE * (Cfg<NP>::D - 1);
+        constexpr int N = (PN_RING_STORES && N0 + EXTRA < 63) ? N0 + EXTRA : (PN_RING_STORES && EXTRA > 0 ? 63 : N0);
 #ifdef PN_TRACE_CHAIN
         const unsigned long long t0 = __builtin_amdgcn_s_memtime();
         asm volatile("s_waitcnt lgkmcnt(0)" ::: "memory");
@@ -413,10 +418,16 @@
 __host__ __device__ constexpr int chunk_steps(int S, int c) {
     return (c == (S - 1) / Cfg<NP>::PER && S % Cfg<NP>::PER) ? S % Cfg<NP>::PER : Cfg<NP>::PER;
 }
-template <int NP, int S, int PP>
+template <int Y_ = 0, int YC_ = 0, int NC_ = 0>
+struct Stores {
+    static constexpr int Y = Y_, YC = YC_, NC = NC_;
+    template <int NP>
+    static constexpr int extra(int chunk) { return (chunk < Cfg<NP>::D ? Y : 0) + (chunk < NC ? YC : 0); }
+};
+template <int NP, int S, int PP, typename YS>
 __device__ __forceinline__ void read_step(Ring<NP>& R, uint32_t& sa, int lane, BFrag<NP>& f) {
     if constexpr (PP < S) {
-        if constexpr (PP % Cfg<NP>::PER == 0) sa = R.acquire() + lane * 16;
+        if constexpr (PP % Cfg<NP>::PER == 0) sa = R.template acquire<YS::template extra<NP>(PP / Cfg<NP>::PER)>() + lane * 16;
         if constexpr (PN_ABL_CHAIN & 2) f = BFrag<NP>{};
         else read_a<NP, PP % Cfg<NP>::PER>(f, sa);
     }
@@ -442,7 +453,7 @@
     v0 = mfma1(a0.p[0], b.p[0], v0);
     v1 = mfma1(a1.p[0], b.p[0], v1);
 }
-template <int NP, int KS, int NT, int S0, bool BIASNEXT, bool ZERO = false>
+template <int NP, int KS, int NT, int S0, bool BIASNEXT, bool ZERO, typename YS>
 struct GemmStep {
     static constexpr int LA = Look<NP>::N, U = Unit<NP, NT>::U;
     static_assert(LA >= U && LA % U == 0 && (KS * NT) % U == 0, "look-ahead in whole units");
@@ -452,8 +463,8 @@
         constexpr int hi = (S0 + LA + U) < S ? (S0 + LA + U) : S;
         constexpr int young = hi > S0 + U ? hi - (S0 + U) : 0;
         BFrag<NP> nw[U];
-        read_step<NP, S, S0 + LA>(R, sa, lane, nw[0]);
-        if constexpr (U == 2) read_step<NP, S, S0 + LA + 1>(R, sa, lane, nw[1]);
+        read_step<NP, S, S0 + LA, YS>(R, sa, lane, nw[0]);
+        if constexpr (U == 2) read_step<NP, S, S0 + LA + 1, YS>(R, sa, lane, nw[1]);
         wait_a<NP, NP * young>(q[0]);
         constexpr int ks = S0 / NT, t = S0 % NT;
         if constexpr (U == 2) {
@@ -486,7 +497,7 @@
             for (int i = 0; i + U < LA; ++i) q[i] = q[i + U];
 #pragma unroll
             for (int u = 0; u < U; ++u) q[LA - U + u] = nw[u];
-            GemmStep<NP, KS, NT, S0 + U, BIASNEXT, ZERO>::run(R, b, acc, sa, q, lane);
+            GemmStep<NP, KS, NT, S0 + U, BIASNEXT, ZERO, YS>::run(R, b, acc, sa, q, lane);
         }
     }
 };
@@ -498,11 +509,11 @@
         gemm_prologue<NP, S, I + 1, BIASNEXT>(R, sa, q);
     }
 }
-template <int NP, int KS, int NT, bool BIAS, bool ZERO, bool BIASNEXT = false>
+template <int NP, int KS, int NT, bool BIAS, bool ZERO, bool BIASNEXT = false, typename YS = Stores<>>
 __device__ __forceinline__ void chain_gemm(Ring<NP>& R, const BFrag<NP> (&b)[KS], accv (&acc)[NT], int lane, int sc = 0) {
     constexpr int CF = Cfg<NP>::CF;
     static_assert(Look<NP>::N <= Cfg<NP>::PER, "the look-ahead stays within one chunk boundary");
-    const uint32_t s0 = R.acquire();
+    const uint32_t s0 = R.template acquire<YS::template extra<NP>(0)>();
     if constexpr (!ZERO && NP == 2) {
 #pragma unroll
         for (int t = 0; t < NT; ++t)
@@ -515,7 +526,7 @@
     uint32_t sa = s0 + lane * 16;
     BFrag<NP> q[Look<NP>::N];
     gemm_prologue<NP, KS * NT, 0, BIASNEXT>(R, sa, q);
-    GemmStep<NP, KS, NT, 0, BIASNEXT, ZERO>::run(R, b, acc, sa, q, lane);
+    GemmStep<NP, KS, NT, 0, BIASNEXT, ZERO, YS>::run(R, b, acc, sa, q, lane);
     if constexpr (BIAS) {
         const float* aux = reinterpret_cast<const float*>(R.lds + ((sa - lane * 16) - R.lds_addr) + CF * 1024) + 4 * (lane / TILE);
         const float inv = NP == 2 ? ldexpf(1.0f, -sc) : 1.0f;
@@ -925,6 +936,20 @@
     store_t<NT>(slot + T.blk * (int64_t)(F * TILE) + opaque(T.lo), acc);
 }
 
+template <int ST>
+__device__ __forceinline__ bool st_keep(bool runtime) { return ST != 0 || runtime; }
+template <int ST>
+__device__ __forceinline__ bool st_q24(int runtime) { return ST == 0 ? runtime != 0 : ST == 2; }
+template <int NP, int ST, int NT>
+constexpr int y_vec() { return (ST == 0 || (PN_ABL_CHAIN & 16)) ? 0 : (ST == 2 && kQ24<NP>) ? NT * ACCQ : 4 * NT * ACCQ; }
+template <int NT>
+constexpr int y_t() { return (PN_ABL_CHAIN & 16) ? 0 : 4 * NT * ACCQ; }
+constexpr int Y_ENC = 96 / QB * 4;
+template <int NP>
+constexpr int short_by(int KS, int NT) {
+    return chunks_of<NP>(KS, NT) < Cfg<NP>::D ? Cfg<NP>::D - chunks_of<NP>(KS, NT) : 0;
+}
+
 template <int NP, int MODE>
 __device__ __forceinline__ Ex encode(const float (&mu)[3], const float (&cv)[3], const float (&vv)[3], int g,
                                       typename TEl<NP>::type* et, BFrag<NP> (&benc)[KS_ENC]) {
@@ -1036,11 +1061,11 @@
         dm[i] = col_sum(dm[i]);
     }
 }
-template <int NP>
+template <int NP, int ST>
 __device__ __forceinline__ Ex finish_gated(accv (&acc)[NT_H], const Gate& m, typename TEl<NP>::type* slot, const Tile& T, bool q24,
                                            BFrag<NP> (&bh)[KS_H]) {
     gate_bits<NT_H>(acc, m);
-    if (slot) store_vec<NP, NT_H>(slot, T, 256, q24, acc);
+    if (st_keep<ST>(slot != nullptr)) store_vec<NP, NT_H>(slot, T, 256, q24, acc);
     return acc_to_b<NP, NT_H, KS_H>(acc, bh, 0.f, EXP_CAP_Z);
 }
 
@@ -1083,7 +1108,7 @@
 }
 __host__ __device__ constexpr int64_t acts_floats(int64_t Mp) { return 8 * Mp * 256 + Mp * 288 + Mp * 128; }
 
-template <int NP>
+template <int NP, int ST>
 __global__ __launch_bounds__(CH_THREADS, CH_MIN_WAVES) void k_chain_fwd(FwdArgs a) {
     extern __shared__ __attribute__((aligned(16))) unsigned char lds[];
     typedef typename TEl<NP>::type TE;
@@ -1130,29 +1155,31 @@
 #endif
             bex = encode<NP, 0>(mu, cv, zero3, T.g, et, benc).ex;
             TR(1);
-            chain_gemm<NP, KS_ENC, NT_H, true, true, true>(R, benc, acc, lane, wx(F_L0) + bex);
+            chain_gemm<NP, KS_ENC, NT_H, true, true, true, Stores<Y_ENC>>(R, benc, acc, lane, wx(F_L0) + bex);
             TR(2);
         }
         auto finish_hidden = [&](int slot) {
             relu<NT_H>(acc);
-            if (TP(a.acts_t)) store_vec<NP, NT_H>(TP(a.acts_t) + act_off(slot, Mp), T, 256, a.q24 && q24_act(slot), acc);
+            if (st_keep<ST>(a.acts_t != nullptr))
+                store_vec<NP, NT_H>(TP(a.acts_t) + act_off(slot, Mp), T, 256, st_q24<ST>(a.q24) && q24_act(slot), acc);
             const Ex e = acc_to_b<NP, NT_H, KS_H>(acc, bh);
             gate_words<NP, KS_H, KS_H>(bh, mw);
             store_gate(a.masks, slot, Mp, T.blk * TILE + T.c, T.g, mw);
             bex = e.ex;
             RM.upd(slot, e.top);
         };
+        typedef Stores<y_vec<NP, ST, NT_H>() + 1> YH;
         finish_hidden(0);
         TR(3);
 #pragma unroll 1
         for (int l = 1; l <= 4; ++l) {
-            chain_gemm<NP, KS_H, NT_H, true, true, true>(R, bh, acc, lane, wx(F_L0 + l) + bex);
+            chain_gemm<NP, KS_H, NT_H, true, true, true, YH>(R, bh, acc, lane, wx(F_L0 + l) + bex);
             TR(2 + 2 * l);
             finish_hidden(l);
             TR(3 + 2 * l);
         }
         {
-            chain_gemm<NP, KS_H, NT_H, false, true, true>(R, bh, acc, lane, wx(F_L5) + bex);
+            chain_gemm<NP, KS_H, NT_H, false, true, true, YH>(R, bh, acc, lane, wx(F_L5) + bex);
             BFrag<NP> benc[KS_ENC];
             const int eex = reload_b<NP, KS_ENC>(et, benc);
             chain_gemm<NP, KS_ENC, NT_H, true, false, true>(R, benc, acc, lane, wx(F_L5E) + eex);
@@ -1162,14 +1189,14 @@
         }
 #pragma unroll 1
         for (int l = 6; l <= 7; ++l) {
-            chain_gemm<NP, KS_H, NT_H, true, true, true>(R, bh, acc, lane, wx(F_L6 + l - 6) + bex);
+            chain_gemm<NP, KS_H, NT_H, true, true, true, YH>(R, bh, acc, lane, wx(F_L6 + l - 6) + bex);
             TR(2 + 2 * l);
             finish_hidden(l);
             TR(3 + 2 * l);
         }
         {
             accv ad[1];
-            chain_gemm<NP, KS_H, 1, true, true, true>(R, bh, ad, lane, wx(F_DEN) + bex);
+            chain_gemm<NP, KS_H, 1, true, true, true, YH>(R, bh, ad, lane, wx(F_DEN) + bex);
             if (T.live) {
 #pragma unroll
                 for (int i = 0; i < 4; ++i) {
@@ -1182,10 +1209,11 @@
         BFrag<NP> bv[KS_H + KS_PAD];
         int vex;
         {
-            chain_gemm<NP, KS_H, NT_H, true, true, true>(R, bh, acc, lane, wx(F_EXTRA) + bex);
+            chain_gemm<NP, KS_H, NT_H, true, true, true, Stores<0, YH::Y, short_by<NP>(KS_H, 1)>>(R, bh, acc, lane, wx(F_EXTRA) + bex);
             TR(19);
-            TE* bt = a.acts_t ? TP(a.acts_t) + act_off(8, Mp) + T.blk * (288 * TILE) + T.lo : nullptr;
-            if (bt) store_t<NT_H>(bt, acc);
+            const bool keep = st_keep<ST>(a.acts_t != nullptr);
+            TE* bt = keep ? TP(a.acts_t) + act_off(8, Mp) + T.blk * (288 * TILE) + T.lo : nullptr;
+            if (keep) store_t<NT_H>(bt, acc);
             const Ex e = acc_to_b<NP, NT_H, KS_H + KS_PAD>(acc, bv, 1.0f);
             vex = e.ex;
             RM.upd(8, e.top);
@@ -1199,7 +1227,7 @@
 #pragma unroll
                     for (int i = 0; i < 4; ++i) {
                         x[4 * h + i] = v[i];
-                        if (bt) bt[(256 + QB * (2 * q + h) + i) * TILE] = (TE)v[i];
+                        if (keep) bt[(256 + QB * (2 * q + h) + i) * TILE] = (TE)v[i];
                     }
                 }
                 split_into<NP>(x, bv[KS_H + q], vex);
@@ -1210,11 +1238,11 @@
         int cex;
         {
             accv av[NT_C];
-            chain_gemm<NP, KS_H + KS_PAD, NT_C, true, true, true>(R, bv, av, lane, wx(F_VIEW) + vex);
+            chain_gemm<NP, KS_H + KS_PAD, NT_C, true, true, true, Stores<ST != 0 ? y_t<NT_H>() + 8 * KS_PAD : 0>>(R, bv, av, lane, wx(F_VIEW) + vex);
             TR(21);
             Gate w4;
             relu<NT_C>(av);
-            if (TP(a.acts_t)) store_t<NT_C>(TP(a.acts_t) + act_off(9, Mp) + T.blk * (128 * TILE) + T.lo, av);
+            if (st_keep<ST>(a.acts_t != nullptr)) store_t<NT_C>(TP(a.acts_t) + act_off(9, Mp) + T.blk * (128 * TILE) + T.lo, av);
             const Ex e = acc_to_b<NP, NT_C, KS_C>(av, bc);
             gate_words<NP, KS_C, KS_C>(bc, w4);
             store_gate(a.masks, 8, Mp, T.blk * TILE + T.c, T.g, w4);
@@ -1224,7 +1252,7 @@
         TR(22);
         {
             accv ac[1];
-            chain_gemm<NP, KS_C, 1, true, true, true>(R, bc, ac, lane, wx(F_COLOR) + cex);
+            chain_gemm<NP, KS_C, 1, true, true, true, Stores<(ST != 0 ? y_t<NT_C>() : 0) + 1>>(R, bc, ac, lane, wx(F_COLOR) + cex);
             TR(23);
             if (T.live && T.g == 0) {
 #pragma unroll
@@ -1268,7 +1296,7 @@
     int q24;
 };
 
-template <int NP>
+template <int NP, int ST>
 __global__ __launch_bounds__(CH_THREADS, CH_MIN_WAVES) void k_chain_dgrad(SweepArgs a) {
     extern __shared__ __attribute__((aligned(16))) unsigned char lds[];
     typedef typename TEl<NP>::type TE;
@@ -1301,11 +1329,13 @@
             else return 0;
         };
         {
-            const bool Q7 = kQ24<NP> && a.q24 && q24_delta(7);
-            TE* rt = (a.keep_all && !Q7) ? TP(a.vec_t) + (int64_t)7 * Mp * 256 + T.blk * (256 * TILE) + T.lo : nullptr;
-            unsigned char* rq = (a.keep_all && Q7) ? reinterpret_cast<unsigned char*>(TP(a.vec_t) + (int64_t)7 * Mp * 256) +
-                                                         T.blk * (int64_t)(256 * TILE * 3) + q24_lane(T.c, T.g)
-                                                   : nullptr;
+            const bool Q7 = kQ24<NP> && st_q24<ST>(a.q24) && q24_delta(7);
+            const bool keep = st_keep<ST>(a.keep_all != 0);
+            const bool st32 = keep && !Q7, st24 = keep && Q7;
+            TE* rt = st32 ? TP(a.vec_t) + (int64_t)7 * Mp * 256 + T.blk * (256 * TILE) + T.lo : nullptr;
+            unsigned char* rq = st24 ? reinterpret_cast<unsigned char*>(TP(a.vec_t) + (int64_t)7 * Mp * 256) +
+                                           T.blk * (int64_t)(256 * TILE * 3) + q24_lane(T.c, T.g)
+                                     : nullptr;
             const Gate m7 = pop_front(mk);
             if constexpr (NP == 2) {
                 float wm = 0.f;
@@ -1329,10 +1359,10 @@
                         const int j = 4 * h + i;
                         const uint32_t bit = (m7.w[gate_word(ks, j)] >> gate_bit(ks, j)) & 1u;
                         x[j] = bit ? sgm * wv[i] : 0.f;
-                        if (rt) rt[(QB * (2 * ks + h) + i) * TILE] = (TE)x[j];
+                        if (st32) rt[(QB * (2 * ks + h) + i) * TILE] = (TE)x[j];
                     }
                     if constexpr (kQ24<NP>) {
-                        if (rq) {
+                        if (st24) {
 #if PN_Q24_NT
                             __builtin_nontemporal_store(pack_q24(x[4 * h], x[4 * h + 1], x[4 * h + 2], x[4 * h + 3]), reinterpret_cast<u32x3*>(rq + (2 * ks + h) * 768));
 #else
@@ -1345,18 +1375,19 @@
             }
         }
         accv acc[NT_H];
+        typedef Stores<y_vec<NP, ST, NT_H>()> YG;
 #pragma unroll 1
         for (int l = 7; l >= 1; --l) {
-            chain_gemm<NP, KS_H, NT_H, false, true>(R, bh, acc, lane, wx(B_L7 + 7 - l) + bex);
-            TE* dst = a.keep_all ? TP(a.vec_t) + (int64_t)(l - 1) * Mp * 256 : (l - 1 == 5 ? TP(a.vec_t) : nullptr);
-            const Ex e = finish_gated<NP>(acc, pop_front(mk), dst, T, a.q24 && q24_delta(l - 1), bh);
+            chain_gemm<NP, KS_H, NT_H, false, true, false, YG>(R, bh, acc, lane, wx(B_L7 + 7 - l) + bex);
+            TE* dst = st_keep<ST>(a.keep_all != 0) ? TP(a.vec_t) + (int64_t)(l - 1) * Mp * 256 : (l - 1 == 5 ? TP(a.vec_t) : nullptr);
+            const Ex e = finish_gated<NP, ST>(acc, pop_front(mk), dst, T, st_q24<ST>(a.q24) && q24_delta(l - 1), bh);
             bex = e.ex;
             RM.upd(l - 1, e.top);
         }
         {
             accv a3[NT_ENC];
-            chain_gemm<NP, KS_H, NT_ENC, false, true>(R, bh, a3, lane, wx(B_DENC0) + bex);
-            bex = reload_b<NP, KS_H>(TP(a.vec_t) + (a.keep_all ? (int64_t)5 * Mp * 256 : 0) + T.blk * (256 * TILE) + T.lo, bh, EXP_CAP_Z);
+            chain_gemm<NP, KS_H, NT_ENC, false, true, false, YG>(R, bh, a3, lane, wx(B_DENC0) + bex);
+            bex = reload_b<NP, KS_H>(TP(a.vec_t) + (st_keep<ST>(a.keep_all != 0) ? (int64_t)5 * Mp * 256 : 0) + T.blk * (256 * TILE) + T.lo, bh, EXP_CAP_Z);
             chain_gemm<NP, KS_H, NT_ENC, false, false>(R, bh, a3, lane, wx(B_DENC1) + bex);
             float dm[3];
             ipe_backward_tiles(a3, mu, cv, T.g, dm);
@@ -1371,7 +1402,7 @@
     if constexpr (NP == 2) RM.flush(a.amax ? a.amax + AM_RS0 : nullptr, lane, wid, lds);
 }
 
-template <int NP>
+template <int NP, int ST>
 __global__ __launch_bounds__(CH_THREADS, CH_MIN_WAVES) void k_chain_tangent(SweepArgs a) {
     extern __shared__ __attribute__((aligned(16))) unsigned char lds[];
     typedef typename TEl<NP>::type TE;
@@ -1411,32 +1442,34 @@
             e = encode<NP, 1>(mu, cv, vv, T.g, et, benc);
             bex = e.ex;
             RM.upd(8, e.top);
-            chain_gemm<NP, KS_ENC, NT_H, false, true>(R, benc, acc, lane, wx(F_L0) + bex);
-        }
-        e = finish_gated<NP>(acc, pop_front(mk), TP(a.vec_t), T, a.q24 && q24_act(0), bh);
+            chain_gemm<NP, KS_ENC, NT_H, false, true, false, Stores<Y_ENC>>(R, benc, acc, lane, wx(F_L0) + bex);
+        }
+        typedef Stores<y_vec<NP, ST, NT_H>()> YG;
+        const bool q24 = st_q24<ST>(a.q24);
+        e = finish_gated<NP, ST>(acc, pop_front(mk), TP(a.vec_t), T, q24 && q24_act(0), bh);
         bex = e.ex;
         RM.upd(0, e.top);
 #pragma unroll 1
         for (int l = 1; l <= 4; ++l) {
-            chain_gemm<NP, KS_H, NT_H, false, true>(R, bh, acc, lane, wx(F_L0 + l) + bex);
-            e = finish_gated<NP>(acc, pop_front(mk), TP(a.vec_t) + (int64_t)l * Mp * 256, T, a.q24 && q24_act(l), bh);
+            chain_gemm<NP, KS_H, NT_H, false, true, false, YG>(R, bh, acc, lane, wx(F_L0 + l) + bex);
+            e = finish_gated<NP, ST>(acc, pop_front(mk), TP(a.vec_t) + (int64_t)l * Mp * 256, T, q24 && q24_act(l), bh);
             bex = e.ex;
             RM.upd(l, e.top);
         }
         {
-            chain_gemm<NP, KS_H, NT_H, false, true>(R, bh, acc, lane, wx(F_L5) + bex);
+            chain_gemm<NP, KS_H, NT_H, false, true, false, YG>(R, bh, acc, lane, wx(F_L5) + bex);
             BFrag<NP> benc[KS_ENC];
             const int eex = reload_b<NP, KS_ENC>(et, benc, EXP_CAP_Z);
             chain_gemm<NP, KS_ENC, NT_H, false, false>(R, benc, acc, lane, wx(F_L5E) + eex);
-            e = finish_gated<NP>(acc, pop_front(mk), TP(a.vec_t) + (int64_t)5 * Mp * 256, T, a.q24 && q24_act(5), bh);
+            e = finish_gated<NP, ST>(acc, pop_front(mk), TP(a.vec_t) + (int64_t)5 * Mp * 256, T, q24 && q24_act(5), bh);
             bex = e.ex;
             RM.upd(5, e.top);
         }
-        chain_gemm<NP, KS_H, NT_H, false, true>(R, bh, acc, lane, wx(F_L6) + bex);
-        e = finish_gated<NP>(acc, pop_front(mk), TP(a.vec_t) + (int64_t)6 * Mp * 256, T, a.q24 && q24_act(6), bh);
+        chain_gemm<NP, KS_H, NT_H, false, true, false, YG>(R, bh, acc, lane, wx(F_L6) + bex);
+        e = finish_gated<NP, ST>(acc, pop_front(mk), TP(a.vec_t) + (int64_t)6 * Mp * 256, T, q24 && q24_act(6), bh);
         bex = e.ex;
         RM.upd(6, e.top);
-        chain_gemm<NP, KS_H, NT_H, false, true>(R, bh, acc, lane, wx(F_L7) + bex);
+        chain_gemm<NP, KS_H, NT_H, false, true, false, YG>(R, bh, acc, lane, wx(F_L7) + bex);
         {
             gate_bits<NT_H>(acc, pop_front(mk));
             store_t<NT_H>(TP(a.vec_t) + (int64_t)7 * Mp * 256 + T.blk * (256 * TILE) + T.lo, acc);
@@ -1480,7 +1513,7 @@
     int q24;
 };
 
-template <int NP>
+template <int NP, int ST>
 __global__ __launch_bounds__(CH_THREADS, CH_MIN_WAVES) void k_chain_bwd(BwdArgs a) {
     extern __shared__ __attribute__((aligned(16))) unsigned char lds[];
     typedef typename TEl<NP>::type TE;
@@ -1527,7 +1560,7 @@
         BFrag<NP> bc[KS_C];
         {
             accv av[NT_C];
-            chain_gemm<NP, 1, NT_C, false, true>(R, b1, av, lane, wx(B_COLOR) + bex);
+            chain_gemm<NP, 1, NT_C, false, true, false, Stores<8>>(R, b1, av, lane, wx(B_COLOR) + bex);
             gate_bits<NT_C>(av, pop_front(mk));
             store_t<NT_C>(TP(a.dhv_t) + T.blk * (128 * TILE) + T.lo, av);
             e = acc_to_b<NP, NT_C, KS_C>(av, bc, 0.f, EXP_CAP_Z);
@@ -1537,7 +1570,7 @@
         BFrag<NP> be[KS_H + 1];
         accv acc[NT_H];
         {
-            chain_gemm<NP, KS_C, NT_H, false, true>(R, bc, acc, lane, wx(B_VIEW) + bex);
+            chain_gemm<NP, KS_C, NT_H, false, true, false, Stores<y_t<NT_C>()>>(R, bc, acc, lane, wx(B_VIEW) + bex);
             TE* bt = TP(a.d8_t) + T.blk * (288 * TILE) + T.lo;
             store_t<NT_H>(bt, acc);
             const float z = a.raw_den[T.rc * a.nc] + a.density_bias;
@@ -1573,14 +1606,16 @@
             }
         }
         BFrag<NP> bh[KS_H];
-        chain_gemm<NP, KS_H + 1, NT_H, false, true>(R, be, acc, lane, wx(B_EXTRA) + bex);
-        e = finish_gated<NP>(acc, pop_front(mk), TP(a.delta_t) + (int64_t)7 * Mp * 256, T, a.q24 && q24_delta(7), bh);
+        chain_gemm<NP, KS_H + 1, NT_H, false, true, false, Stores<y_t<NT_H>() + 8>>(R, be, acc, lane, wx(B_EXTRA) + bex);
+        typedef Stores<y_vec<NP, ST, NT_H>()> YG;
+        const bool q24 = st_q24<ST>(a.q24);
+        e = finish_gated<NP, ST>(acc, pop_front(mk), TP(a.delta_t) + (int64_t)7 * Mp * 256, T, q24 && q24_delta(7), bh);
         bex = e.ex;
         RM.upd(7, e.top);
 #pragma unroll 1
         for (int l = 7; l >= 1; --l) {
-            chain_gemm<NP, KS_H, NT_H, false, true>(R, bh, acc, lane, wx(B_L7 + 7 - l) + bex);
-            e = finish_gated<NP>(acc, pop_front(mk), TP(a.delta_t) + (int64_t)(l - 1) * Mp * 256, T, a.q24 && q24_delta(l - 1), bh);
+            chain_gemm<NP, KS_H, NT_H, false, true, false, YG>(R, bh, acc, lane, wx(B_L7 + 7 - l) + bex);
+            e = finish_gated<NP, ST>(acc, pop_front(mk), TP(a.delta_t) + (int64_t)(l - 1) * Mp * 256, T, q24 && q24_delta(l - 1), bh);
             bex = e.ex;
             RM.upd(l - 1, e.top);
         }
@@ -1592,7 +1627,7 @@
                 cv[i] = a.cov[T.rc * 3 + i];
             }
             accv a3[NT_ENC];
-            chain_gemm<NP, KS_H, NT_ENC, false, true>(R, bh, a3, lane, wx(B_DENC0) + bex);
+            chain_gemm<NP, KS_H, NT_ENC, false, true, false, YG>(R, bh, a3, lane, wx(B_DENC0) + bex);
             bex = reload_b<NP, KS_H>(TP(a.delta_t) + (int64_t)5 * Mp * 256 + T.blk * (256 * TILE) + T.lo, bh, EXP_CAP_Z);
             chain_gemm<NP, KS_H, NT_ENC, false, false>(R, bh, a3, lane, wx(B_DENC1) + bex);
             float dm[3];
@@ -2340,14 +2375,47 @@
     PN_CHECK_LAUNCH();
     return PN_OK;
 }
-#define LAUNCH_CHAIN(KERNEL, planes, nst, wgs, args, s, cls, flops)                                                   \
-    do {                                                                                                             \
-        static AttrDone done3 = {}, done2 = {}, done1 = {};                                                          \
-        if ((planes) == 3) return launch_chain(KERNEL<3>, Cfg<3>::LDS_BYTES, done3, nst, wgs, args, s, cls, flops);  \
-        if ((planes) == 2) return launch_chain(KERNEL<2>, Cfg<2>::LDS_BYTES, done2, nst, wgs, args, s, cls, flops);  \
-        if ((planes) == 1) return launch_chain(KERNEL<1>, Cfg<1>::LDS_BYTES, done1, nst, wgs, args, s, cls, flops);  \
-        return PN_ERR_UNSUPPORTED;                                                                                   \
+#define LAUNCH_CHAIN_ST(KERNEL, NP_, ST_, nst, wgs, args, s, cls, flops)                                 \
+    do {                                                                                                 \
+        static AttrDone done = {};                                                                       \
+        return launch_chain(KERNEL<NP_, ST_>, Cfg<NP_>::LDS_BYTES, done, nst, wgs, args, s, cls, flops); \
     } while (0)
+#if PN_RING_STORES
+#define LAUNCH_CHAIN_ST0_OPT(KERNEL, NP_, keep, nst, wgs, args, s, cls, flops) \
+    if (!(keep)) LAUNCH_CHAIN_ST(KERNEL, NP_, 0, nst, wgs, args, s, cls, flops)
+#define LAUNCH_CHAIN_ST0_ALWAYS(KERNEL, NP_, keep, nst, wgs, args, s, cls, flops)
+#if PN_CHAIN_TILE == 16 && !PN_NO_Q24
+#define LAUNCH_CHAIN_ST2(KERNEL, q24, nst, wgs, args, s, cls, flops) \
+    if (q24) LAUNCH_CHAIN_ST(KERNEL, 2, 2, nst, wgs, args, s, cls, flops)
+#else
+#define LAUNCH_CHAIN_ST2(KERNEL, q24, nst, wgs, args, s, cls, flops)
+#endif
+#define LAUNCH_CHAIN(KERNEL, planes, keep, OPT, q24, nst, wgs, args, s, cls, flops)            \
+    do {                                                                                       \
+        if ((planes) == 3) {                                                                   \
+            LAUNCH_CHAIN_ST0##OPT(KERNEL, 3, keep, nst, wgs, args, s, cls, flops);             \
+            LAUNCH_CHAIN_ST(KERNEL, 3, 1, nst, wgs, args, s, cls, flops);                      \
+        }                                                                                      \
+        if ((planes) == 2) {                                                                   \
+            LAUNCH_CHAIN_ST0##OPT(KERNEL, 2, keep, nst, wgs, args, s, cls, flops);             \
+            LAUNCH_CHAIN_ST2(KERNEL, q24, nst, wgs, args, s, cls, flops);                      \
+            LAUNCH_CHAIN_ST(KERNEL, 2, 1, nst, wgs, args, s, cls, flops);                      \
+        }                                                                                      \
+        if ((planes) == 1) {                                                                   \
+            LAUNCH_CHAIN_ST0##OPT(KERNEL, 1, keep, nst, wgs, args, s, cls, flops);             \
+            LAUNCH_CHAIN_ST(KERNEL, 1, 1, nst, wgs, args, s, cls, flops);                      \
+        }                                                                                      \
+        return PN_ERR_UNSUPPORTED;                                                             \
+    } while (0)
+#else
+#define LAUNCH_CHAIN(KERNEL, planes, keep, OPT, q24, nst, wgs, args, s, cls, flops)            \
+    do {                                                                                       \
+        if ((planes) == 3) LAUNCH_CHAIN_ST(KERNEL, 3, 0, nst, wgs, args, s, cls, flops);       \
+        if ((planes) == 2) LAUNCH_CHAIN_ST(KERNEL, 2, 0, nst, wgs, args, s, cls, flops);       \
+        if ((planes) == 1) LAUNCH_CHAIN_ST(KERNEL, 1, 0, nst, wgs, args, s, cls, flops);       \
+        return PN_ERR_UNSUPPORTED;                                                             \
+    } while (0)
+#endif
 struct ChainGeom {
     int64_t slot, bytes;
     int f_all, f_den, b_all, b_l7, b_denc0;
@@ -2578,7 +2646,7 @@
     hipLaunchKernelGGL(k_view_table, dim3((unsigned)((view_rows * 32 + 255) / 256)), dim3(256), 0, (hipStream_t)stream, view_rows,
                        viewdirs, view_tab, a.amax, AM_COUNT);
     PN_CHECK_LAUNCH();
-    LAUNCH_CHAIN(k_chain_fwd, planes, a.nst, max_wgs, a, (hipStream_t)stream, 2, (double)M * flops_mlp(nc));
+    LAUNCH_CHAIN(k_chain_fwd, planes, acts_t != nullptr, _OPT, t_format != 0, a.nst, max_wgs, a, (hipStream_t)stream, 2, (double)M * flops_mlp(nc));
 }
 
 int pn_chain_density_grad(int64_t M, int nc, int planes, float density_bias, const float* params, const void* pack,
@@ -2603,7 +2671,7 @@
     a.vec_t = rs_t; a.out3 = grad_mean; a.keep_all = keep_all != 0;
     a.amax = planes == 2 ? amax : nullptr;
     a.q24 = t_format;
-    LAUNCH_CHAIN(k_chain_dgrad, planes, a.nst, max_wgs, a, (hipStream_t)stream, 3, (double)M * kFlopsSweep);
+    LAUNCH_CHAIN(k_chain_dgrad, planes, keep_all != 0, _OPT, t_format != 0, a.nst, max_wgs, a, (hipStream_t)stream, 3, (double)M * kFlopsSweep);
 }
 
 int pn_chain_tangent(int64_t M, int nc, int planes, const float* params, const void* pack, const float* mean,
@@ -2627,7 +2695,7 @@
     a.vec_t = tang_t; a.edot_t = edot_t; a.sdot = sdot;
     a.amax = planes == 2 ? amax : nullptr;
     a.q24 = t_format;
-    LAUNCH_CHAIN(k_chain_tangent, planes, a.nst, max_wgs, a, (hipStream_t)stream, 4, (double)M * kFlopsSweep);
+    LAUNCH_CHAIN(k_chain_tangent, planes, true, _ALWAYS, t_format != 0, a.nst, max_wgs, a, (hipStream_t)stream, 4, (double)M * kFlopsSweep);
 }
 
 int pn_chain_backward(int64_t M, int nc, int planes, float density_bias, const void* pack, const uint32_t* masks,
@@ -2655,7 +2723,7 @@
     a.drgb_t = drgb_t; a.dhv_t = dhv_t; a.d8_t = d8_t; a.delta_t = delta_t; a.coef_t = coef_t; a.d_mean = d_mean;
     a.amax = planes == 2 ? amax : nullptr;
     a.q24 = t_format;
-    LAUNCH_CHAIN(k_chain_bwd, planes, a.nst, max_wgs, a, (hipStream_t)stream, 5, (double)M * (flops_mlp(nc) - (d_mean ? 0.0 : 2.0 * 2 * 96 * 256)));
+    LAUNCH_CHAIN(k_chain_bwd, planes, true, _ALWAYS, t_format != 0, a.nst, max_wgs, a, (hipStream_t)stream, 5, (double)M * (flops_mlp(nc) - (d_mean ? 0.0 : 2.0 * 2 * 96 * 256)));
 }
 
 
```

Result: no change. 186,500, median of 6 (+0.2%).
